# itxtx/normalizing-flows-study

Measured on AMD Instinct MI355X. Metric: log_prob samples/sec/GPU + test-NLL match; RealNVP d=2 and MAF d=63, higher is better.
Workload: dtype fp32

## Files before the change

### include/nfx.h

```cpp
#ifndef NFX_H
#define NFX_H

#include <stddef.h>
#include <stdint.h>

#ifdef __cplusplus
extern "C" {
#endif

#define NFX_ABI_VERSION 3

#define NFX_OK 0
#define NFX_EINVAL (-1)
#define NFX_EUNSUPPORTED (-2)
#define NFX_ELAUNCH (-3)

#define NFX_FORWARD 1
#define NFX_INVERSE (-1)

#define NFX_MAF_INVERSE 0
#define NFX_IAF_FORWARD 1
#define NFX_MAF_FORWARD 2
#define NFX_IAF_INVERSE 3

typedef struct NfxMlpRaw {
    const float* w[4];
    const float* b[4];
    const float* mask[4];
    const float* bn_w[3];
    const float* bn_b[3];
    const float* bn_rm[3];
    const float* bn_rv[3];
    float bn_eps;
    int n_layers;
} NfxMlpRaw;

int nfx_abi_version(void);
const char* nfx_last_error(void);
const char* nfx_last_kernel(void);
int nfx_debug_fill_lds(uint32_t bits, void* stream);

size_t nfx_affine_packed_floats(int d, int H);
int nfx_affine_pack(const NfxMlpRaw* s_net, const NfxMlpRaw* b_net, const float* mask, int d,
                    int H, float* packed, void* stream);
int nfx_affine_coupling(const float* packed, const float* in, float* out, float* log_det,
                        int64_t B, int d, int H, int direction, int accumulate, void* stream);
int nfx_affine_coupling_logprob(const float* packed, const float* in, float* out, float* log_det,
                                float* logp, double* sums, void* workspace, int64_t B, int d,
                                int H, int accumulate, void* stream);
#define NFX_AFFINE_AUTO 0
#define NFX_AFFINE_STREAMING 1
#define NFX_AFFINE_SMALL 2
int nfx_affine_kernel_policy(int policy);

int nfx_affine_chain_supported(int64_t B, int d, int H);
int nfx_affine_chain(const float* const* packs, int n_layers, const float* in, float* out,
                     float* log_det, int64_t B, int d, int H, int direction, int accumulate,
                     void* stream);
int nfx_affine_chain_logprob(const float* const* packs, int n_layers, const float* in, float* out,
                             float* log_det, float* logp, double* sums, void* workspace, int64_t B,
                             int d, int H, int accumulate, void* stream);
int nfx_affine_chain_sample(const float* const* packs, int n_layers, uint64_t seed, uint64_t* rng_state,
                            float* z, float* x, float* log_det, int64_t B, int d, int H, void* stream);

size_t nfx_spline_packed_floats(int d, int H, int K);
int nfx_spline_pack(const NfxMlpRaw* param_net, const float* mask, int d, int H, int K,
                    float* packed, void* stream);
int nfx_spline_coupling(const float* packed, const float* in, float* out, float* log_det,
                        int64_t B, int d, int H, int K, float bound, float min_bin_width,
                        float min_bin_height, float min_derivative, int rescale,
                        float data_min, float data_max, int direction, int accumulate,
                        void* stream);
int nfx_spline_coupling_logprob(const float* packed, const float* in, float* out, float* log_det,
                                float* logp, double* sums, void* workspace, int64_t B, int d,
                                int H, int K, float bound, float min_bin_width,
                                float min_bin_height, float min_derivative, int rescale,
                                float data_min, float data_max, int accumulate, void* stream);

int nfx_spline_chain_supported(int64_t B, int d, int H, int K);
int nfx_spline_chain(const float* const* packs, int n_layers, const float* in, float* out, float* log_det,
                     int64_t B, int d, int H, int K, float bound, float min_bin_width, float min_bin_height,
                     float min_derivative, int direction, int accumulate, void* stream);
int nfx_spline_chain_logprob(const float* const* packs, int n_layers, const float* in, float* out,
                             float* log_det, float* logp, double* sums, void* workspace, int64_t B, int d,
                             int H, int K, float bound, float min_bin_width, float min_bin_height,
                             float min_derivative, int accumulate, void* stream);
int nfx_spline_chain_sample(const float* const* packs, int n_layers, uint64_t seed, uint64_t* rng_state,
                            float* z, float* x, float* log_det, int64_t B, int d, int H, int K, float bound,
                            float min_bin_width, float min_bin_height, float min_derivative, void* stream);

int nfx_rqs_unit(const float* in, const float* widths, const float* heights,
                 const float* derivatives, float* out, float* log_det, int64_t N, int K,
                 float min_bin_width, float min_bin_height, float min_derivative, int inverse,
                 void* stream);
int nfx_rqs_unit_backward(const float* in, const float* widths, const float* heights,
                          const float* derivatives, const float* grad_out, const float* grad_log_det,
                          float* grad_in, float* grad_widths, float* grad_heights, float* grad_derivatives,
                          int64_t N, int K, float min_bin_width, float min_bin_height, float min_derivative,
                          int inverse, void* stream);

size_t nfx_arqs_packed_floats(int d, int H, int K);
int nfx_arqs_pack(const NfxMlpRaw* made, int d, int H, int K, float* packed, void* stream);
int nfx_arqs(const float* packed, const float* in, float* out, float* log_det, int64_t B, int d,
             int H, int K, float min_bin_width, float min_bin_height, float min_derivative,
             int rescale, double data_min, double data_max, int direction, int accumulate,
             void* stream);

int nfx_base_normal(uint64_t seed, uint64_t* rng_state, float* z, int64_t B, int d, void* stream);

size_t nfx_made_packed_floats(int d, int H);
int nfx_made_pack(const NfxMlpRaw* net, int d, int H, float* packed, void* stream);
int nfx_made_pack_parallel(const NfxMlpRaw* net, int d, int H, float* packed, void* stream);
int nfx_made_pack_sequential(int d, int H, float* packed, void* stream);
int nfx_made_affine(const float* packed, const float* in, float* out, float* log_det,
                    int64_t B, int d, int H, int variant, int accumulate, void* stream);
#define NFX_MADE_SEQ_AUTO 0
#define NFX_MADE_SEQ_SEGMENT 1
#define NFX_MADE_SEQ_WAVE 2
#define NFX_MADE_SEQ_PUSH 3
int nfx_made_seq_policy(int policy);
int nfx_made_affine_logprob(const float* packed, const float* in, float* out, float* log_det,
                            float* logp, double* sums, void* workspace, int64_t B, int d, int H,
                            int variant, int accumulate, void* stream);
int nfx_made_sample_supported(int d, int H, int variant);
int nfx_made_affine_sample(const float* packed, uint64_t seed, uint64_t* rng_state, float* z, float* x,
                           float* log_det, int64_t B, int d, int H, void* stream);

int nfx_made_pack_backward(const NfxMlpRaw* net, int d, int H, float* packed, void* stream);
size_t nfx_made_backward_factor_floats(int64_t B, int d, int H);
int64_t nfx_made_backward_max_batch(int d, int H);
int nfx_made_affine_backward(const float* packed, const float* in, const float* grad_out,
                             const float* grad_log_det, float* grad_in, float* factors, int64_t B,
                             int d, int H, int variant, void* stream);

int nfx_made_seq_backward(const float* packed, const float* in, const float* grad_out,
                          const float* grad_log_det, float* grad_in, float* factors, int64_t B,
                          int d, int H, int variant, void* stream);
int64_t nfx_made_factor_pitch(int64_t B);
size_t nfx_made_param_floats(int d, int H);
size_t nfx_made_wgrad_workspace_bytes(int64_t B, int d, int H);
int nfx_made_backward_weights(const float* factors, int64_t B, int d, int H,
                              const float* const* masks, float* grads, void* workspace,
                              void* stream);

size_t nfx_spline_backward_packed_floats(int d, int H, int K);
size_t nfx_spline_backward_param_floats(int d, int H, int K);
size_t nfx_spline_backward_workspace_bytes(int64_t B, int d, int H, int K);
int nfx_spline_pack_backward(const NfxMlpRaw* net, const float* mask, int d, int H, int K,
                             float* packed, void* stream);
int nfx_spline_coupling_backward(const float* packed, const float* mask, const float* in,
                                 const float* grad_out, const float* grad_log_det, float* grad_in,
                                 float* grads, void* workspace, int64_t B, int d, int H, int K,
                                 int n_transformed, float bound, float min_bin_width,
                                 float min_bin_height, float min_derivative, int direction,
                                 void* stream);

size_t nfx_affine_train_pack_floats(int d, int H);
size_t nfx_affine_train_stats_doubles(int H);
size_t nfx_affine_train_grad_doubles(int d, int H);
size_t nfx_affine_train_param_floats(int d, int H);
size_t nfx_affine_train_workspace_bytes(int64_t B, int d, int H);
int nfx_affine_train_pack(const NfxMlpRaw* s_net, const NfxMlpRaw* b_net, const float* mask,
                          const double* stats1, const double* stats2, int d, int H, float* tpack,
                          float* epack, void* stream);
int nfx_affine_train_stats(const float* tpack, const float* in, int64_t B, int d, int H, int layer,
                           double* stats, void* workspace, void* stream);
int nfx_affine_train_update_running(const double* stats1, const double* stats2,
                                    float* const* running_mean, float* const* running_var, int H,
                                    double momentum, void* stream);
int nfx_affine_train_update_running_counted(const double* stats1, const double* stats2,
                                            float* const* running_mean, float* const* running_var,
                                            int64_t* const* num_batches_tracked, int H,
                                            double momentum, void* stream);
int nfx_affine_train_backward(const float* tpack, const float* in, const float* grad_out,
                              const float* grad_log_det, float* grad_in, int64_t B, int d, int H,
                              int direction, int stage, const double* stats2, double* G,
                              void* workspace, void* stream);
int nfx_affine_train_assemble(const double* G, const double* stats1, const double* stats2, int d,
                              int H, float eps, float* grads, void* stream);
size_t nfx_affine_train_keep_floats(int64_t B, int d, int H);
int nfx_affine_train_stats_keep(const float* tpack, const float* in, int64_t B, int d, int H,
                                int layer, double* stats, void* workspace, float* keep,
                                void* stream);
int nfx_affine_train_backward_keep(const float* tpack, const float* in, const float* grad_out,
                                   const float* grad_log_det, float* grad_in, int64_t B, int d,
                                   int H, int direction, int stage, const double* stats2,
                                   double* G, void* workspace, const float* keep, void* stream);
int nfx_affine_train_output(const float* tpack, const float* in, const float* keep, float* out,
                            float* log_det, int64_t B, int d, int H, int direction, void* stream);
int nfx_affine_eval_stats(float* const* running_mean, float* const* running_var, int H,
                          double* stats1, double* stats2, void* stream);

size_t nfx_gauss_workspace_bytes(int64_t B);
int nfx_gauss_workspace_init(void* workspace, void* stream);
int nfx_gauss_logprob(const float* z, const float* log_det, float* logp, double* sums,
                      void* workspace, int64_t B, int d, void* stream);
int nfx_gauss_logprob_backward(const float* z, const float* grad_logp, float* grad_z, float* grad_log_det,
                               int64_t B, int d, void* stream);

size_t nfx_flowbn_workspace_bytes(int64_t B, int d);
int nfx_flowbn_apply(const float* in, float* out, float* log_det, const float* gamma, const float* beta,
                     const float* running_mean, const float* running_var, float eps, int64_t B, int d,
                     int direction, void* stream);
int nfx_flowbn_moments(const float* x, int64_t B, int d, double* stats, void* workspace, void* stream);
int nfx_flowbn_update_running(const double* stats, float* running_mean, float* running_var,
                              double momentum, int d, void* stream);
int nfx_flowbn_backward(const float* in, const float* grad_out, const float* grad_log_det, float* grad_in,
                        const float* gamma, const float* beta, const float* running_mean,
                        const float* running_var, float eps, float* grad_gamma, float* grad_beta,
                        int64_t B, int d, int direction, void* workspace, void* stream);


int nfx_linear_forward(const float* x, const float* w, const float* wmask, const float* b, const float* in_scale,
                       const float* post_scale, const float* post_shift, float* y, int64_t M, int K, int N,
                       int relu, void* stream);
int nfx_linear_backward_data(const float* gy, const float* w, const float* wmask, const float* act,
                             const float* out_scale, float* gx, int64_t M, int N, int K, int accumulate, void* stream);
size_t nfx_linear_workspace_bytes(int64_t M, int N, int K);
int nfx_linear_backward_weight(const float* gy, const float* x, const float* in_scale, const float* wmask, float* gw,
                               float* gb, int64_t M, int N, int K, void* workspace, void* stream);
int nfx_made_elem_forward(const float* x, const float* params, float* y, float* log_det, int64_t B, int d,
                          int variant, int accumulate, void* stream);
int nfx_made_elem_step(const float* x, const float* params, float* work, float* work_ld, int64_t B, int d, int i,
                       int variant, void* stream);
int nfx_made_elem_finish(const float* x, const float* work, const float* work_ld, float* y, float* log_det,
                         int64_t B, int d, int variant, int accumulate, void* stream);
int nfx_made_elem_backward(const float* x, const float* params, const float* gy, const float* gld, float* gparams,
                           float* gx, int64_t B, int d, int variant, void* stream);
int nfx_made_elem_seq_backward(const float* x, const float* params, const float* work, const float* lam,
                               const float* gy, const float* gld, float* out, int64_t B, int d, int variant, int mode,
                               void* stream);
int nfx_made_elem_seq_step_backward(const float* x, const float* params, const float* work, const float* work_ld,
                                    const float* lam, const float* grad_out, const float* grad_log_det,
                                    float* grad_params, float* grad_in, int64_t B, int d, int i, int variant,
                                    void* stream);
int nfx_made_elem_prefix(const float* work, float* out, int64_t B, int d, int i, void* stream);
int nfx_affine_elem_forward(const float* x, const float* s_raw, const float* b_raw, const float* mask, float* y,
                            float* log_det, int64_t B, int d, int direction, int accumulate, void* stream);
int nfx_affine_elem_backward(const float* x, const float* s_raw, const float* b_raw, const float* mask,
                             const float* gy, const float* gld, float* gs, float* gb, float* gx, int64_t B, int d,
                             int direction, void* stream);
int nfx_bn_prepare(const double* stats, const float* gamma, const float* beta, float* running_mean,
                   float* running_var, double eps, double momentum, int update_running, int N, float* mean,
                   float* invstd, float* scale, float* shift, void* stream);
int nfx_bn_apply_relu(const float* z, const float* scale, const float* shift, float* h, int64_t M, int N,
                      void* stream);
size_t nfx_bn_workspace_bytes(int64_t M, int N);
int nfx_bn_backward_sums(const float* g, const float* z, const float* mean, const float* invstd, double* sums,
                         int64_t M, int N, void* workspace, void* stream);
int nfx_bn_backward_apply(const float* g, const float* z, const float* mean, const float* invstd,
                          const float* gamma, const double* sums, const double* count, int train, float* gz,
                          int64_t M, int N, void* stream);
int nfx_arqs_step(const float* xr, const float* params, float* state, float* log_det, const float* gld, float* lam,
                  float* gparams, float* gx, int64_t B, int d, int K, int i, int direction, int mode,
                  float min_bin_width, float min_bin_height, float min_derivative, void* stream);
int nfx_arqs_bounds(const float* in, const float* bounds, float* out, int64_t B, int d, int mode, void* stream);
int nfx_spline_elem_forward(const float* x, const float* params, const float* mask, float* y, float* log_det,
                            int64_t B, int d, int K, float bound, float min_bin_width, float min_bin_height,
                            float min_derivative, int direction, int accumulate, void* stream);
int nfx_spline_elem_backward(const float* x, const float* params, const float* mask, const float* gy,
                             const float* gld, float* gparams, float* gx, int64_t B, int d, int K, float bound,
                             float min_bin_width, float min_bin_height, float min_derivative, int direction,
                             void* stream);
int nfx_spline_elem_forward_bounded(const float* x, const float* params, const float* mask, const float* bounds,
                                    float* y, float* log_det, int64_t B, int d, int K, float bound,
                                    float min_bin_width, float min_bin_height, float min_derivative, int direction,
                                    int accumulate, void* stream);
int nfx_spline_elem_backward_bounded(const float* x, const float* params, const float* mask, const float* bounds,
                                     const float* gy, const float* gld, float* gparams, float* gx, int64_t B, int d,
                                     int K, float bound, float min_bin_width, float min_bin_height,
                                     float min_derivative, int direction, void* stream);
int nfx_spline_rescale(const float* x, const float* bounds, float* xr, int64_t B, int d, float bound, void* stream);

size_t nfx_cnf_packed_floats(int d, int H);
int nfx_cnf_pack(const float* w1, const float* b1, const float* w2, const float* b2, const float* w3,
                 const float* b3, int d, int H, float* packed, void* stream);
int nfx_cnf_supported(int64_t B, int d, int H);
int nfx_cnf_integrate(const float* packed, const float* in, float* out, float* log_det, int64_t B, int d,
                      int H, float t_begin, float t_end, float step_size, int accumulate, void* stream);

int nfx_cnf_backward_supported(int64_t B, int d, int H);
size_t nfx_cnf_backward_packed_floats(int d, int H);
size_t nfx_cnf_trajectory_floats(int64_t B, int d, float t_begin, float t_end, float step_size);
size_t nfx_cnf_backward_workspace_floats(int64_t B, int d, int H);
size_t nfx_cnf_backward_slots(int64_t B, int d, int H);
size_t nfx_cnf_backward_block_threads(int64_t B, int d, int H);
int nfx_cnf_pack_backward(const float* w1, const float* b1, const float* w2, const float* b2, const float* w3,
                          const float* b3, int d, int H, float* packed, void* stream);
int nfx_cnf_integrate_save(const float* packed, const float* in, float* out, float* log_det, float* traj,
                           int64_t B, int d, int H, float t_begin, float t_end, float step_size, int accumulate,
                           void* stream);
int nfx_cnf_backward(const float* packed, const float* w1, const float* w2, const float* w3, const float* in,
                     const float* traj, const float* gy, const float* gld, float* gx, float* gw1, float* gb1,
                     float* gw2, float* gb2, float* gw3, float* gb3, float* workspace, int64_t B, int d, int H,
                     float t_begin, float t_end, float step_size, void* stream);

#define NFX_RESIDUAL_RELU 0
#define NFX_RESIDUAL_ELU 1
#define NFX_RESIDUAL_LEAKY_RELU 2
#define NFX_RESIDUAL_TANH 3
size_t nfx_residual_packed_floats(int d, int H);
int nfx_residual_supported(int64_t B, int d, int H, int activation);
int nfx_residual_pack(const float* w1, const float* b1, const float* u1, const float* v1, float c1, const float* w2,
                      const float* b2, const float* u2, const float* v2, float c2, const float* w3, const float* b3,
                      const float* u3, const float* v3, float c3, int d, int H, float* packed, void* stream);
int nfx_residual_flow(const float* packed, const float* in, float* out, float* log_det, int64_t B, int d, int H,
                      int activation, int direction, int neumann_terms, int max_iter, float tol, int accumulate,
                      void* stream);

int nfx_residual_backward_supported(int64_t B, int d, int H, int activation);
size_t nfx_residual_backward_packed_floats(int d, int H);
size_t nfx_residual_backward_workspace_floats(int64_t B, int d, int H);
size_t nfx_residual_backward_slots(int64_t B, int d, int H);
size_t nfx_residual_backward_block_threads(int64_t B, int d, int H);
int nfx_residual_pack_backward(const float* w1, const float* b1, const float* u1, const float* v1, float c1,
                               const float* w2, const float* b2, const float* u2, const float* v2, float c2,
                               const float* w3, const float* b3, const float* u3, const float* v3, float c3, int d,
                               int H, float* packed, void* stream);
int nfx_residual_backward(const float* packed, const float* z, const float* gy, const float* gld, float* gx,
                          float* gw1, float* gb1, float* gw2, float* gb2, float* gw3, float* gb3, float* workspace,
                          int64_t B, int d, int H, int activation, int direction, int neumann_terms, void* stream);

#define NFX_NAF_RELU 0
#define NFX_NAF_ELU 1
#define NFX_NAF_LEAKY_RELU 2
#define NFX_NAF_GELU 3
#define NFX_NAF_LAYER_NORM 1
#define NFX_NAF_RESIDUAL(l) (2 << (l))
typedef struct NfxNafLayer {
    const float* weight;
    const float* bias;
    const float* mask;
    const float* ln_weight;
    const float* ln_bias;
    float ln_eps;
    int residual;
} NfxNafLayer;
size_t nfx_naf_packed_floats(int d, int n_hidden, const int* widths);
int nfx_naf_supported(int64_t B, int d, int n_hidden, const int* widths, int activation, int flags);
int nfx_naf_pack(const NfxNafLayer* layers, int d, int n_hidden, const int* widths, float* packed, void* stream);
int nfx_naf_flow(const float* packed, const float* in, float* out, float* log_det, int64_t B, int d, int n_hidden,
                 const int* widths, int activation, int flags, float clamp_alpha, float clamp_log_scale,
                 int direction, int accumulate, void* stream);

typedef struct NfxNafLayerGrad {
    float* weight;
    float* bias;
    float* ln_weight;
    float* ln_bias;
} NfxNafLayerGrad;
int nfx_naf_backward_supported(int64_t B, int d, int n_hidden, const int* widths, int activation, int flags);
size_t nfx_naf_backward_packed_floats(int d, int n_hidden, const int* widths);
int nfx_naf_pack_backward(const NfxNafLayer* layers, int d, int n_hidden, const int* widths, float* packed,
                          void* stream);
size_t nfx_naf_backward_slots(int64_t B, int d, int n_hidden, const int* widths);
size_t nfx_naf_backward_block_threads(int64_t B, int d, int n_hidden, const int* widths);
size_t nfx_naf_backward_workspace_floats(int64_t B, int d, int n_hidden, const int* widths);
int nfx_naf_backward(const float* packed, const NfxNafLayer* layers, const float* x, const float* gz,
                     const float* gld, float* gx, const NfxNafLayerGrad* grads, float* workspace, int64_t B, int d,
                     int n_hidden, const int* widths, int activation, int flags, float clamp_alpha,
                     float clamp_log_scale, void* stream);

int nfx_lowrank_supported(int64_t B, int dim, int n_layers);
size_t nfx_lowrank_record_floats(int dim);
int nfx_lowrank_pack_planar(const float* w, const float* u_hat, const float* b, int dim, int max_iter, float tol,
                            float* record, void* stream);
int nfx_lowrank_pack_radial(const float* z0, const float* alpha_hat, const float* beta_hat, int dim, int max_iter,
                            float tol, float* record, void* stream);
int nfx_lowrank_pack_sylvester(const float* v, const float* R, const float* b, int dim, int num_householder,
                               int num_transforms, int max_iter, float tol, float* record, void* stream);
int nfx_lowrank_stack(const float* image, int n_layers, const float* x, float* out, float* log_det, int64_t B,
                      int dim, int direction, int accumulate, void* stream);

int nfx_lrbwd_supported(int64_t B, int dim, int n_layers, int direction);
size_t nfx_lrbwd_max_layers(int dim);
size_t nfx_lrbwd_chunk_rows(int dim);
size_t nfx_lrbwd_slots(int64_t B, int dim, int n_layers);
size_t nfx_lrbwd_workspace_floats(int64_t B, int dim, int n_layers);
int nfx_lrbwd_stack(const float* image, int n_layers, const float* point, const float* gv, const float* gld, float* gx,
                    float* workspace, int64_t B, int dim, int direction, void* stream);
int nfx_lrbwd_param_grads(const float* workspace, int64_t B, int dim, int n_layers, int layer, int kind,
                          const float* p0, const float* p1, const float* p2, float* g0, float* g1, float* g2,
                          int num_householder, int num_transforms, void* stream);

#ifdef __cplusplus
}
#endif

#endif
```

### normalizing-flows-study_amd/csrc/nfx_affine_kernel.h

```cpp
#pragma once
#include <type_traits>
#include <utility>

#include "nfx_common.h"

namespace nfx {

__host__ __device__ constexpr int up4(int v) { return (v + 3) & ~3; }

struct AffineLayout {
    int d, HT, KS1;
    int w1, b1, w2, b2, w3, b3, net, mask, total;
    int s;
};

constexpr uint32_t kAffineLiveElide = 0x100u;
struct AffineSplit {
    int w1, b1, b2, w3, b3, w2s, net, mask, ok, total;
};

__host__ __device__ constexpr AffineSplit affine_split(int d, int HT) {
    AffineSplit S{};
    int o = 0;
    S.w1 = o; o += HT * ((d + 1) / 2) * 64;
    S.b1 = o; o += HT * 32;
    S.b2 = o; o += HT * 32;
    S.w3 = o; o += d * HT * 32;
    S.b3 = o; o += up4(d);
    S.w2s = o; o += HT * 2 * HT * 768;
    S.net = o;
    S.mask = 2 * o;
    S.ok = S.mask + up4(d);
    S.total = S.ok + 4;
    return S;
}

__host__ __device__ constexpr bool affine_has_split(int d, int HT) { return d <= 8 && HT <= 2; }

__host__ __device__ constexpr AffineLayout affine_layout(int d, int HT) {
    AffineLayout L{};
    L.d = d;
    L.HT = HT;
    L.KS1 = (d + 1) / 2;
    int o = 0;
    L.w1 = o; o += HT * L.KS1 * 64;
    L.b1 = o; o += HT * 32;
    L.w2 = o; o += HT * HT * 16 * 64;
    L.b2 = o; o += HT * 32;
    if (d <= 8) {
        L.w3 = o; o += d * HT * 32;
        L.b3 = o; o += up4(d);
    } else {
        const int NJ = (d + 31) / 32;
        L.w3 = o; o += NJ * HT * 1024;
        L.b3 = o; o += NJ * 32;
    }
    L.net = o;
    L.mask = 2 * o;
    L.total = 2 * o + up4(d);
    L.s = L.total;
    if (affine_has_split(d, HT)) L.total += affine_split(d, HT).total;
    return L;
}

template <int D>
__device__ __forceinline__ void load_row(const float* __restrict__ p, float (&v)[D]) {
    if constexpr (D == 2) {
        float2 t = *reinterpret_cast<const float2*>(p);
        v[0] = t.x; v[1] = t.y;
    } else if constexpr (D == 4) {
        float4 t = *reinterpret_cast<const float4*>(p);
        v[0] = t.x; v[1] = t.y; v[2] = t.z; v[3] = t.w;
    } else {
#pragma unroll
        for (int j = 0; j < D; ++j) v[j] = p[j];
    }
}

template <int D>
__device__ __forceinline__ void store_row(float* __restrict__ p, const float (&v)[D]) {
    if constexpr (D == 2) {
        *reinterpret_cast<float2*>(p) = make_float2(v[0], v[1]);
    } else if constexpr (D == 4) {
        *reinterpret_cast<float4*>(p) = make_float4(v[0], v[1], v[2], v[3]);
    } else {
#pragma unroll
        for (int j = 0; j < D; ++j) p[j] = v[j];
    }
}

template <int HT, int D, int TILES = 2>
__device__ __forceinline__ void affine_net(const float* __restrict__ P, const AffineLayout& L,
                                           const float (&xb)[2][(D + 1) / 2], float (&res)[D]) {
    constexpr int KS1 = (D + 1) / 2;
    const int lane = lane_id(), h = lane >> 5;

    f32x16 h1[HT][2];
#pragma unroll
    for (int ht = 0; ht < HT; ++ht) {
        f32x16 a0, a1;
        load_bias16_x2(P + L.b1 + ht * 32, h, a0, a1);
#pragma unroll
        for (int ks = 0; ks < KS1; ++ks) {
            const float w = P[L.w1 + (ht * KS1 + ks) * 64 + lane];
            a0 = mfma32(w, xb[0][ks], a0);
            if constexpr (TILES == 2) a1 = mfma32(w, xb[1][ks], a1);
        }
#pragma unroll
        for (int r = 0; r < 16; ++r) {
            a0[r] = trelu(a0[r]);
            if constexpr (TILES == 2) a1[r] = trelu(a1[r]);
        }
        h1[ht][0] = a0;
        h1[ht][1] = a1;
    }

    float part[D][2];
#pragma unroll
    for (int j = 0; j < D; ++j) part[j][0] = part[j][1] = 0.f;
    const f32x4* wg = reinterpret_cast<const f32x4*>(P + L.w2) + lane;
#pragma unroll
    for (int hto = 0; hto < HT; ++hto) {
        f32x16 a0, a1;
        load_bias16_x2(P + L.b2 + hto * 32, h, a0, a1);
#pragma unroll
        for (int kt = 0; kt < HT; ++kt) {
#pragma unroll
            for (int rq = 0; rq < 4; ++rq) {
                const f32x4 w = wg[a_quad(a_tile(hto, kt, HT), rq) * 64];
#pragma unroll
                for (int rr = 0; rr < 4; ++rr) {
                    a0 = mfma32(w[rr], h1[kt][0][4 * rq + rr], a0);
                    if constexpr (TILES == 2) a1 = mfma32(w[rr], h1[kt][1][4 * rq + rr], a1);
                }
            }
        }
#pragma unroll
        for (int j = 0; j < D; ++j) {
            const f32x16 w3 = load_bias16(P + L.w3 + (j * HT + hto) * 32, h);
#pragma unroll
            for (int r = 0; r < 16; ++r) {
                part[j][0] = fmaf(w3[r], trelu(a0[r]), part[j][0]);
                if constexpr (TILES == 2) part[j][1] = fmaf(w3[r], trelu(a1[r]), part[j][1]);
            }
        }
    }
#pragma unroll
    for (int j = 0; j < D; ++j)
        res[j] = tclamp(halves_sum(part[j][0], part[j][1]) + P[L.b3 + j], -10.f, 10.f);
}

#ifndef NFX_SPLIT_TERMS
#define NFX_SPLIT_TERMS 6
#endif
typedef __bf16 bf16x8 __attribute__((ext_vector_type(8)));
typedef uint32_t u32x4 __attribute__((ext_vector_type(4)));

__device__ __forceinline__ f32x16 mfma_bf16(u32x4 a, u32x4 b, f32x16 c) {
    return __builtin_amdgcn_mfma_f32_32x32x16_bf16(__builtin_bit_cast(bf16x8, a), __builtin_bit_cast(bf16x8, b), c,
                                                    0, 0, 0);
}

__device__ __forceinline__ void split3(float x, uint32_t& u0, uint32_t& u1, uint32_t& u2) {
    u0 = __float_as_uint(x) & 0xffff0000u;
    const float r1 = x - __uint_as_float(u0);
    u1 = __float_as_uint(r1) & 0xffff0000u;
    u2 = __float_as_uint(r1 - __uint_as_float(u1));
}

__device__ __forceinline__ uint32_t pack_bf16(uint32_t lo, uint32_t hi) {
    return __builtin_amdgcn_perm(hi, lo, 0x07060302u);
}

__device__ __forceinline__ void split_block(const f32x16& a, int half, u32x4 (&xp)[3]) {
#pragma unroll
    for (int q = 0; q < 4; ++q) {
        uint32_t l0, l1, l2, h0, h1, h2;
        split3(a[8 * half + 2 * q], l0, l1, l2);
        split3(a[8 * half + 2 * q + 1], h0, h1, h2);
        xp[0][q] = pack_bf16(l0, h0);
        xp[1][q] = pack_bf16(l1, h1);
        xp[2][q] = pack_bf16(l2, h2);
    }
}

template <class F, int... I>
__device__ __forceinline__ void static_for_seq(F&& f, std::integer_sequence<int, I...>) {
    (f(std::integral_constant<int, I>{}), ...);
}
template <int N, class F>
__device__ __forceinline__ void static_for(F&& f) {
    static_for_seq(f, std::make_integer_sequence<int, N>{});
}

#if NFX_SPLIT_TERMS == 8
constexpr int kSplitTermW[8] = {2, 1, 2, 1, 0, 1, 0, 0}, kSplitTermX[8] = {1, 2, 0, 1, 2, 0, 1, 0};
#else
constexpr int kSplitTermW[6] = {2, 1, 0, 1, 0, 0}, kSplitTermX[6] = {0, 1, 2, 0, 1, 0};
#endif

template <int HT, int D, int TILES, bool LIVE>
__device__ __forceinline__ void affine_nets_split_pipe(const float* __restrict__ S, const AffineSplit& SL,
                                                       const float (&xb)[2][(D + 1) / 2], float (&sv)[D],
                                                       float (&bv)[D], uint32_t live_idx) {
    constexpr int KS1 = (D + 1) / 2;
    constexpr int NJ = LIVE ? (D + 1) / 2 : D;
    constexpr int NS = 2 * TILES;
    constexpr int KB = 2 * HT;
    constexpr int NT = NFX_SPLIT_TERMS;
    constexpr int NM = NT * HT;
    constexpr int NG = KB * NM;
    constexpr int NFI = 16 * HT;
    constexpr int NQ = 3 * HT;
    constexpr int WG0 = (NM - NQ) / 2;
    constexpr int L1G = (KB - 2) * NM;
    constexpr int L1P = L1G >= 2 ? L1G - 2 : 0;
    constexpr int HB0 = NM / 2;
    const int lane = lane_id(), h = lane >> 5;

    const float* Sn[NS];
    const u32x4* w2n[NS];
    f32x16 h1[NS][HT];
    uint32_t u[NS * KB][3][8];
    u32x4 xp[NS * KB][3];
    u32x4 w[NS * KB][HT][3];
    f32x16 hi[NS][HT], lo[NS][HT];
    f32x4 w3q[NS][HT][NJ][4];
    float r1[NS * KB][8], tf[NS][NFI];
    float part[2][NJ][2];
    int w3row[NJ];
#pragma unroll
    for (int j = 0; j < NJ; ++j) w3row[j] = (LIVE ? (int)((live_idx >> (4 * j)) & 7u) : j) * HT * 32;
#pragma unroll
    for (int n = 0; n < 2; ++n)
#pragma unroll
        for (int j = 0; j < NJ; ++j) part[n][j][0] = part[n][j][1] = 0.f;

    auto base = [&](int s) __attribute__((always_inline)) {
        Sn[s] = S + (s / TILES) * SL.net + opaque_zero();
        w2n[s] = reinterpret_cast<const u32x4*>(Sn[s] + SL.w2s) + lane;
    };
    auto l1_bias = [&](int s) __attribute__((always_inline)) {
#pragma unroll
        for (int ht = 0; ht < HT; ++ht) h1[s][ht] = load_bias16(Sn[s] + SL.b1 + ht * 32, h);
    };
    auto l1_mfma = [&](int s) __attribute__((always_inline)) {
#pragma unroll
        for (int ht = 0; ht < HT; ++ht)
#pragma unroll
            for (int ks = 0; ks < KS1; ++ks)
                h1[s][ht] = mfma32(Sn[s][SL.w1 + (ht * KS1 + ks) * 64 + lane], xb[s % TILES][ks], h1[s][ht]);
    };
    auto split_slot = [&](int b, int i) __attribute__((always_inline)) {
        const int s = b / KB, kb = b % KB, q = i / 3;
#pragma unroll
        for (int e = 2 * q; e < 2 * q + 2; ++e) {
            if (i % 3 == 0) {
                const float x = trelu(h1[s][kb >> 1][8 * (kb & 1) + e]);
                u[b][0][e] = __float_as_uint(x) & 0xffff0000u;
                r1[b][e] = x - __uint_as_float(u[b][0][e]);
            } else if (i % 3 == 1) {
                u[b][1][e] = __float_as_uint(r1[b][e]) & 0xffff0000u;
                u[b][2][e] = __float_as_uint(r1[b][e] - __uint_as_float(u[b][1][e]));
            }
        }
        if (i % 3 == 2) {
#pragma unroll
            for (int p = 0; p < 3; ++p) xp[b][p][q] = pack_bf16(u[b][p][2 * q], u[b][p][2 * q + 1]);
        }
    };
    auto w2_quad = [&](int b, int i) __attribute__((always_inline)) {
        const int s = b / KB, kb = b % KB, p = 2 - i / HT, hto = i % HT;
        w[b][hto][p] = w2n[s][((hto * KB + kb) * 3 + p) * 64];
    };
    auto w3_quads = [&](int s, int hto, int rq) __attribute__((always_inline)) {
#pragma unroll
        for (int j = 0; j < NJ; ++j)
            w3q[s][hto][j][rq] = *reinterpret_cast<const f32x4*>(Sn[s] + SL.w3 + w3row[j] + hto * 32 + 16 * h + 4 * rq);
    };
    auto fold_relu = [&](int s, int f) __attribute__((always_inline)) {
        tf[s][f] = trelu(hi[s][f / 16][f % 16] + lo[s][f / 16][f % 16]);
    };
    auto fold_fma = [&](int s, int f) __attribute__((always_inline)) {
        const int hto = f / 16, r = f % 16;
#pragma unroll
        for (int j = 0; j < NJ; ++j)
            part[s / TILES][j][s % TILES] = fmaf(w3q[s][hto][j][r / 4][r % 4], tf[s][f], part[s / TILES][j][s % TILES]);
    };
    constexpr auto fold_gap = [](int f) { return (((f | 1) + 1) * NG + NFI - 1) / NFI - 1; };
    constexpr auto w3_gap = [](int f) {
        const int g = (((f | 1) + 1) * NG + NFI - 1) / NFI - 1;
        return g >= 2 ? g - 2 : 0;
    };
    static_assert(fold_gap(NFI - 1) < NG && fold_gap(0) >= 1 && w3_gap(0) < fold_gap(0), "fold schedule");
    static_assert(WG0 >= 0 && WG0 + NQ <= NM && HB0 + HT <= NM - HT, "read schedule");
    static_assert(KB < 2 || L1G <= (KB - 1) * NM - 1, "layer 1 of the next stage precedes its first split");

    base(0);
    l1_bias(0);
#pragma unroll
    for (int i = 0; i < NQ; ++i) w2_quad(0, i);
    l1_mfma(0);
#pragma unroll
    for (int i = 0; i < 12; ++i) split_slot(0, i);

    static_for<NS>([&](auto sc) __attribute__((always_inline)) {
        constexpr int s = decltype(sc)::value;
        static_for<NG>([&](auto gc) __attribute__((always_inline)) {
            constexpr int g = decltype(gc)::value;
            constexpr int kb = g / NM, m = g % NM, b = s * KB + kb;
            constexpr int t = m / HT, hto = m % HT;
            __builtin_amdgcn_sched_barrier(0);
            if (t == NT - 1) {
                hi[s][hto] = mfma_bf16(w[b][hto][kSplitTermW[t]], xp[b][kSplitTermX[t]], hi[s][hto]);
            } else {
                lo[s][hto] = mfma_bf16(w[b][hto][kSplitTermW[t]], xp[b][kSplitTermX[t]],
                                       kb == 0 && t == 0 ? f32x16{} : lo[s][hto]);
            }
            __builtin_amdgcn_sched_barrier(0);
            if (g == 0 && s + 1 < NS) base(s + 1);
            if (b + 1 < NS * KB && m >= WG0 && m < WG0 + NQ) w2_quad(b + 1, m - WG0);
            if (kb == 0 && m >= HB0 && m < HB0 + HT)
                hi[s][m - HB0] = load_bias16(Sn[s] + SL.b2 + (m - HB0) * 32, h);
            if (s > 0) {
#pragma unroll
                for (int fq = 0; fq < NFI; fq += 4)
                    if (w3_gap(fq) == g) w3_quads(s - 1, fq / 16, (fq % 16) / 4);
            }
            if (s + 1 < NS && g == L1P) l1_bias(s + 1);
            if (s + 1 < NS && g == L1G) l1_mfma(s + 1);
            if (b + 1 < NS * KB) {
#pragma unroll
                for (int i = m * 12 / NM; i < (m + 1) * 12 / NM; ++i) split_slot(b + 1, i);
            }
            if (s > 0) {
#pragma unroll
                for (int f = 0; f < NFI; ++f)
                    if ((fold_gap(f) >= 1 ? fold_gap(f) - 1 : 0) == g) fold_relu(s - 1, f);
#pragma unroll
                for (int f = 0; f < NFI; ++f)
                    if (fold_gap(f) == g) fold_fma(s - 1, f);
            }
        });
    });
    __builtin_amdgcn_sched_barrier(0);
#pragma unroll
    for (int fq = 0; fq < NFI; fq += 4) w3_quads(NS - 1, fq / 16, (fq % 16) / 4);
#pragma unroll
    for (int f = 0; f < NFI; ++f) {
        fold_relu(NS - 1, f);
        fold_fma(NS - 1, f);
    }
    if constexpr (LIVE) {
#pragma unroll
        for (int j = 0; j < D; ++j) sv[j] = bv[j] = 0.f;
#pragma unroll
        for (int jj = 0; jj < NJ; ++jj) {
            const int o = (int)((live_idx >> (4 * jj)) & 15u);
            const float s = tclamp(halves_sum(part[0][jj][0], part[0][jj][1]) + Sn[0][SL.b3 + (o & 7)], -10.f, 10.f);
            const float b = tclamp(halves_sum(part[1][jj][0], part[1][jj][1]) + Sn[NS - 1][SL.b3 + (o & 7)], -10.f, 10.f);
#pragma unroll
            for (int j = 0; j < D; ++j) {
                sv[j] = o == j ? s : sv[j];
                bv[j] = o == j ? b : bv[j];
            }
        }
    } else {
#pragma unroll
        for (int j = 0; j < D; ++j) {
            sv[j] = tclamp(halves_sum(part[0][j][0], part[0][j][1]) + Sn[0][SL.b3 + j], -10.f, 10.f);
            bv[j] = tclamp(halves_sum(part[1][j][0], part[1][j][1]) + Sn[NS - 1][SL.b3 + j], -10.f, 10.f);
        }
    }
}

template <int KS1>
__device__ __forceinline__ bool affine_live_unit(const float (&xb)[2][KS1], const float (&mkb)[KS1]) {
    bool bad = false;
#pragma unroll
    for (int st = 0; st < 2; ++st)
#pragma unroll
        for (int ks = 0; ks < KS1; ++ks)
            bad = bad || (mkb[ks] == 1.f && (!(fabsf(xb[st][ks]) <= 1e33f) || __float_as_uint(xb[st][ks]) == 0x80000000u));
    return __builtin_amdgcn_ballot_w64(bad) == 0;
}

template <int HT, int D, int TILES = 2>
__device__ __forceinline__ void affine_net_split(const float* __restrict__ S, const AffineSplit& SL,
                                                 const float (&xb)[2][(D + 1) / 2], float (&res)[D]) {
    constexpr int KS1 = (D + 1) / 2;
    const int lane = lane_id(), h = lane >> 5;

    f32x16 h1[HT][2];
#pragma unroll
    for (int ht = 0; ht < HT; ++ht) {
        f32x16 a0, a1;
        load_bias16_x2(S + SL.b1 + ht * 32, h, a0, a1);
#pragma unroll
        for (int ks = 0; ks < KS1; ++ks) {
            const float w = S[SL.w1 + (ht * KS1 + ks) * 64 + lane];
            a0 = mfma32(w, xb[0][ks], a0);
            if constexpr (TILES == 2) a1 = mfma32(w, xb[1][ks], a1);
        }
#pragma unroll
        for (int r = 0; r < 16; ++r) {
            a0[r] = trelu(a0[r]);
            if constexpr (TILES == 2) a1[r] = trelu(a1[r]);
        }
        h1[ht][0] = a0;
        h1[ht][1] = a1;
    }

    float part[D][2];
#pragma unroll
    for (int j = 0; j < D; ++j) part[j][0] = part[j][1] = 0.f;
    auto fold = [&](int hto, const f32x16& a, int st) {
#pragma unroll
        for (int j = 0; j < D; ++j) {
            const f32x16 w3 = load_bias16(S + SL.w3 + (j * HT + hto) * 32, h);
#pragma unroll
            for (int r = 0; r < 16; ++r) part[j][st] = fmaf(w3[r], trelu(a[r]), part[j][st]);
        }
    };
    const u32x4* w2s = reinterpret_cast<const u32x4*>(S + SL.w2s) + lane;
#pragma unroll
    for (int st = 0; st < TILES; ++st) {
        u32x4 xp[2 * HT][3];
#pragma unroll
        for (int kb = 0; kb < 2 * HT; ++kb) split_block(h1[kb >> 1][st], kb & 1, xp[kb]);
        const u32x4* w2 = w2s + opaque_zero();
#pragma unroll
        for (int hto = 0; hto < HT; ++hto) {
            f32x16 hi = load_bias16(S + SL.b2 + hto * 32 + opaque_zero(), h), lo = {};
#pragma unroll
            for (int kb = 0; kb < 2 * HT; ++kb) {
                const int g = (hto * 2 * HT + kb) * 3;
                const u32x4 w[3] = {w2[g * 64], w2[(g + 1) * 64], w2[(g + 2) * 64]};
#if NFX_SPLIT_TERMS == 8
                lo = mfma_bf16(w[2], xp[kb][1], lo);
                lo = mfma_bf16(w[1], xp[kb][2], lo);
#endif
                lo = mfma_bf16(w[2], xp[kb][0], lo);
                lo = mfma_bf16(w[1], xp[kb][1], lo);
                lo = mfma_bf16(w[0], xp[kb][2], lo);
                lo = mfma_bf16(w[1], xp[kb][0], lo);
                lo = mfma_bf16(w[0], xp[kb][1], lo);
                hi = mfma_bf16(w[0], xp[kb][0], hi);
            }
            fold(hto, hi + lo, st);
        }
    }
#pragma unroll
    for (int j = 0; j < D; ++j)
        res[j] = tclamp(halves_sum(part[j][0], part[j][1]) + S[SL.b3 + j], -10.f, 10.f);
}

__host__ __device__ constexpr bool affine_split_piped(int HT, int D) { return HT == 2 && D <= 4; }

template <int HT, int D, int TILES, bool PIPE>
__device__ __forceinline__ void affine_nets_split(const float* __restrict__ S, const AffineSplit& SL,
                                                  const float* __restrict__ Pg, const AffineLayout& L,
                                                  const float (&xb)[2][(D + 1) / 2], float (&sv)[D], float (&bv)[D],
                                                  bool live = false, uint32_t live_idx = 0) {
    constexpr int KS1 = (D + 1) / 2;
    const bool wok = S[SL.ok] != 0.f;
    const float xs = S[SL.ok + 1];
    bool fast[2];
#pragma unroll
    for (int st = 0; st < 2; ++st) {
        bool bad = false;
#pragma unroll
        for (int ks = 0; ks < KS1; ++ks) bad = bad || !(fabsf(xb[st][ks]) <= xs);
        fast[st] = wok && __builtin_amdgcn_ballot_w64(bad) == 0;
    }
    if constexpr (PIPE) {
        bool full = !live;
        if (live) {
            affine_nets_split_pipe<HT, D, TILES, true>(S, SL, xb, sv, bv, live_idx);
            bool zero = true;
#pragma unroll
            for (int j = 0; j < D; ++j) zero = zero && fabsf(sv[j]) < 1e-30f;
            full = __builtin_amdgcn_ballot_w64(zero) != 0;
        }
        if (full) affine_nets_split_pipe<HT, D, TILES, false>(S, SL, xb, sv, bv, 0u);
    } else {
        affine_net_split<HT, D, TILES>(S, SL, xb, sv);
        __builtin_amdgcn_sched_barrier(0);
        affine_net_split<HT, D, TILES>(S + SL.net, SL, xb, bv);
    }
    if (!(fast[0] && (TILES == 1 || fast[1]))) {
        __builtin_amdgcn_sched_barrier(0);
        const float* P = Pg + opaque_zero();
        float s2[D], b2[D];
        affine_net<HT, D, TILES>(P, L, xb, s2);
        __builtin_amdgcn_sched_barrier(0);
        affine_net<HT, D, TILES>(P + L.net, L, xb, b2);
        if (!fast[lane_id() >> 5]) {
#pragma unroll
            for (int j = 0; j < D; ++j) {
                sv[j] = s2[j];
                bv[j] = b2[j];
            }
        }
    }
}

template <int HT, int D, int DIR, bool LOGP>
__global__ __launch_bounds__(256) void affine_coupling_kernel(
    const float* __restrict__ packed, const float* __restrict__ in, float* __restrict__ out,
    float* __restrict__ logdet, int64_t B, int accumulate, int64_t nchunks,
    float* __restrict__ logp, double* __restrict__ partials, double* __restrict__ sums, float cgauss) {
    constexpr AffineLayout L = affine_layout(D, HT);
    constexpr int KS1 = L.KS1;
    constexpr bool SPLIT = affine_has_split(D, HT);
    constexpr AffineSplit SL = affine_split(D, HT);
    constexpr int MASK = SPLIT ? SL.mask : L.mask;
    extern __shared__ f32x4 lds4[];
    {
        const f32x4* src = reinterpret_cast<const f32x4*>(packed + (SPLIT ? L.s : 0));
        for (int i = threadIdx.x; i < (SPLIT ? SL.total : L.total) / 4; i += 256) lds4[i] = src[i];
    }
    __syncthreads();
    const float* sm = reinterpret_cast<const float*>(lds4);

    const int lane = lane_id(), h = lane >> 5, col = lane & 31;
    const int64_t nwaves = (int64_t)gridDim.x * 4;
    float mk[D], mkb[KS1];
#pragma unroll
    for (int j = 0; j < D; ++j) mk[j] = sm[MASK + j];
#pragma unroll
    for (int ks = 0; ks < KS1; ++ks) mkb[ks] = (2 * ks + h < D) ? sm[MASK + 2 * ks + h] : 0.f;
    const int64_t wv = (int64_t)blockIdx.x * 4 + (threadIdx.x >> 6);
    const int64_t F = nchunks / nwaves, R = nchunks - F * nwaves;
    const bool split = 2 * R <= nwaves;
    const int64_t nfull = split ? F : F + (wv < R ? 1 : 0);
    const bool half = split && wv < 2 * R;
    const int64_t half_base = F * nwaves * 64 + wv * 32;

    struct Fetch {
        float xb[2][KS1];
        float xr[D];
        float ldin;
    };
    auto fetch = [&](int64_t u, Fetch& f) {
        const int64_t base = u < nfull ? (wv + u * nwaves) * 64 : half_base;
        const int nsamp = u < nfull ? 64 : (u == nfull && half ? 32 : 0);
#pragma unroll
        for (int st = 0; st < 2; ++st) {
            const int64_t s = base + 32 * st + col;
#pragma unroll
            for (int ks = 0; ks < KS1; ++ks) {
                const int k = 2 * ks + h;
                f.xb[st][ks] = (32 * st + col < nsamp && k < D && s < B) ? in[s * D + k] : 0.f;
            }
        }
        const int64_t so = base + lane;
        if (lane < nsamp && so < B) {
            load_row<D>(in + so * D, f.xr);
            f.ldin = accumulate ? logdet[so] : 0.f;
        } else {
#pragma unroll
            for (int j = 0; j < D; ++j) f.xr[j] = 0.f;
            f.ldin = 0.f;
        }
    };

    double lpacc = 0.0;
    auto unit = [&](auto tiles_c, int64_t base, const Fetch& cur) {
        constexpr int TILES = decltype(tiles_c)::value;
        const float* smi = sm + opaque_zero();
        float xb[2][KS1];
#pragma unroll
        for (int st = 0; st < 2; ++st) {
#pragma unroll
            for (int ks = 0; ks < KS1; ++ks) xb[st][ks] = cur.xb[st][ks] * mkb[ks];
        }

        float sv[D], bv[D];
        if constexpr (SPLIT) {
            affine_nets_split<HT, D, TILES, false>(smi, SL, packed, L, xb, sv, bv);
        } else {
            affine_net<HT, D, TILES>(smi, L, xb, sv);
            affine_net<HT, D, TILES>(smi + L.net, L, xb, bv);
        }

        const int64_t so = base + lane;
        if (lane < 32 * TILES && so < B) {
#pragma clang fp contract(off)
            float y[D];
            float ld = 0.f;
#pragma unroll
            for (int j = 0; j < D; ++j) {
                const float m = mk[j], om = 1.f - m;
                const float xa = cur.xr[j] * m;
                float t;
                if constexpr (DIR < 0) {
                    t = (cur.xr[j] - bv[j]) * exp_fast(-sv[j]);
                    ld = ld + om * (-sv[j]);
                } else {
                    t = cur.xr[j] * exp_fast(sv[j]) + bv[j];
                    ld = ld + om * sv[j];
                }
                const float v = xa + om * t;
                y[j] = nonfinite(v) ? 0.f : v;
            }
            if (nonfinite(ld)) ld = 0.f;
            store_row<D>(out + so * D, y);
            const float ldt = accumulate ? cur.ldin + ld : ld;
            logdet[so] = ldt;
            if constexpr (LOGP) {
                float m = gauss_sq0(y[0]);
#pragma unroll
                for (int j = 1; j < D; ++j) m = gauss_sq(m, y[j]);
                const float lp = gauss_lp(m, cgauss, ldt);
                logp[so] = lp;
                lpacc += (double)lp;
            }
        }
    };

    Fetch cur;
    fetch(0, cur);
    for (int64_t u = 0; u < nfull; ++u) {
        Fetch nxt;
        fetch(u + 1, nxt);
        unit(std::integral_constant<int, 2>{}, (wv + u * nwaves) * 64, cur);
        cur = nxt;
    }
    if (half) unit(std::integral_constant<int, 1>{}, half_base, cur);
    if constexpr (LOGP) {
        logp_commit<256>(lpacc, partials, sums, B);
    }
}


constexpr int kWideWaves = 4;

template <int HT>
__device__ __forceinline__ void wide_net(const float* __restrict__ P, const AffineLayout& L, const float* xt, int S,
                                         const float* __restrict__ mask, int d, f32x16 (&res)[2]) {
    const int lane = lane_id(), h = lane >> 5, col = lane & 31;
    f32x16 h1[HT];
#pragma unroll
    for (int ht = 0; ht < HT; ++ht) h1[ht] = load_bias16(P + L.b1 + ht * 32, h);
    for (int ks = 0; ks < L.KS1; ++ks) {
        const int k = 2 * ks + h;
        const float xb = k < d ? xt[col * S + k] * mask[k] : 0.f;
#pragma unroll
        for (int ht = 0; ht < HT; ++ht) h1[ht] = mfma32(P[L.w1 + (ht * L.KS1 + ks) * 64 + lane], xb, h1[ht]);
    }
#pragma unroll
    for (int ht = 0; ht < HT; ++ht)
#pragma unroll
        for (int r = 0; r < 16; ++r) h1[ht][r] = trelu(h1[ht][r]);
    f32x16 h2[HT];
#pragma unroll
    for (int hto = 0; hto < HT; ++hto) {
        f32x16 a = load_bias16(P + L.b2 + hto * 32, h);
#pragma unroll
        for (int kt = 0; kt < HT; ++kt)
#pragma unroll
            for (int rq = 0; rq < 4; ++rq) {
                const f32x4 w = *reinterpret_cast<const f32x4*>(P + L.w2 + (a_quad(a_tile(hto, kt, HT), rq) * 64 + lane) * 4);
#pragma unroll
                for (int rr = 0; rr < 4; ++rr) a = mfma32(w[rr], h1[kt][4 * rq + rr], a);
            }
#pragma unroll
        for (int r = 0; r < 16; ++r) a[r] = trelu(a[r]);
        h2[hto] = a;
    }
    const int NJ = (d + 31) / 32;
#pragma unroll
    for (int j = 0; j < 2; ++j) {
        if (j < NJ) {
            f32x16 a = load_bias16(P + L.b3 + j * 32, h);
#pragma unroll
            for (int kt = 0; kt < HT; ++kt)
#pragma unroll
                for (int rq = 0; rq < 4; ++rq) {
                    const f32x4 w = *reinterpret_cast<const f32x4*>(P + L.w3 + (a_quad(a_tile(j, kt, HT), rq) * 64 + lane) * 4);
#pragma unroll
                    for (int rr = 0; rr < 4; ++rr) a = mfma32(w[rr], h2[kt][4 * rq + rr], a);
                }
#pragma unroll
            for (int r = 0; r < 16; ++r) a[r] = tclamp(a[r], -10.f, 10.f);
            res[j] = a;
        } else {
            res[j] = f32x16{};
        }
    }
}

template <int HT, int DIR, bool LOGP>
__global__ __launch_bounds__(64 * kWideWaves) void affine_wide_kernel(
    const float* __restrict__ packed, const float* __restrict__ in, float* __restrict__ out,
    float* __restrict__ logdet, int64_t B, int d, int accumulate, int64_t ntiles,
    float* __restrict__ logp, double* __restrict__ partials, double* __restrict__ sums, float cgauss) {
    const AffineLayout L = affine_layout(d, HT);
    const int S = d | 1;
    extern __shared__ f32x4 lds4[];
    const int wave = __builtin_amdgcn_readfirstlane(threadIdx.x >> 6);
    float* xt = reinterpret_cast<float*>(lds4) + wave * 32 * S;
    const int lane = lane_id(), h = lane >> 5, col = lane & 31;
    const float* mask = packed + L.mask;
    double lpacc = 0.0;
    for (int64_t t = (int64_t)blockIdx.x * kWideWaves + wave; t < ntiles; t += (int64_t)gridDim.x * kWideWaves) {
        const int64_t base = t * 32;
        const int rows = (int)(B - base < 32 ? B - base : 32);
        const float* src = in + base * d;
        for (int i = lane; i < 32 * d; i += 64) {
            const int r = i / d, c = i - r * d;
            xt[r * S + c] = r < rows ? src[i] : 0.f;
        }
        const float ldin = (accumulate && lane < rows) ? logdet[base + lane] : 0.f;
        wave_lds_sync();
        const float* Pw = packed + opaque_zero();
        f32x16 sv[2], bv[2];
        wide_net<HT>(Pw, L, xt, S, mask, d, sv);
        wide_net<HT>(Pw + L.net, L, xt, S, mask, d, bv);
        float ldp = 0.f;
        {
#pragma clang fp contract(off)
#pragma unroll
            for (int j = 0; j < 2; ++j)
#pragma unroll
                for (int r = 0; r < 16; ++r) {
                    const int dim = 32 * j + crow(r, h);
                    if (dim < d) {
                        float* px = xt + col * S + dim;
                        const float xv = *px, m = mask[dim], om = 1.f - m;
                        float tv;
                        if constexpr (DIR < 0) {
                            tv = (xv - bv[j][r]) * exp_fast(-sv[j][r]);
                            ldp = ldp + om * (-sv[j][r]);
                        } else {
                            tv = xv * exp_fast(sv[j][r]) + bv[j][r];
                            ldp = ldp + om * sv[j][r];
                        }
                        const float v = xv * m + om * tv;
                        *px = nonfinite(v) ? 0.f : v;
                    }
                }
        }
        float ld = halves_sum(ldp, ldp);
        if (nonfinite(ld)) ld = 0.f;
        wave_lds_sync();
        float* dst = out + base * d;
        for (int i = lane; i < rows * d; i += 64) {
            const int r = i / d, c = i - r * d;
            dst[i] = xt[r * S + c];
        }
        if (lane < rows) {
            const float ldt = accumulate ? ldin + ld : ld;
            logdet[base + lane] = ldt;
            if constexpr (LOGP) {
                float m = gauss_sq0(xt[lane * S]);
                for (int c = 1; c < d; ++c) m = gauss_sq(m, xt[lane * S + c]);
                const float lp = gauss_lp(m, cgauss, ldt);
                logp[base + lane] = lp;
                lpacc += (double)lp;
            }
        }
        wave_lds_sync();
    }
    if constexpr (LOGP) {
        logp_commit<64 * kWideWaves>(lpacc, partials, sums, B);
    }
}

typedef void (*affine_kernel_t)(const float*, const float*, float*, float*, int64_t, int, int64_t,
                                float*, double*, double*, float);

template <int HT>
affine_kernel_t affine_pick_ht(int d, int dir, bool logp);

template <int HT>
affine_kernel_t affine_pick(int d, int dir, bool logp) {
    return pick_range<1, 8>(d, [=](auto D) -> affine_kernel_t {
        if (dir > 0) return affine_coupling_kernel<HT, D(), 1, false>;
        return logp ? affine_coupling_kernel<HT, D(), -1, true> : affine_coupling_kernel<HT, D(), -1, false>;
    });
}

int affine_split_pack(float* packed, int d, int H, hipStream_t s);

}
```

### normalizing-flows-study_amd/csrc/nfx_made.hip

```cpp
#include "nfx_made_kernel.h"
#include "nfx_made_wide_kernel.h"
#include <atomic>
#include <cstdlib>

#include "nfx_made_seqs_kernel.h"
#include "nfx_pack.h"

namespace nfx {

__global__ void made_pack_kernel(NfxMlpRaw net, int d, int H, float* packed) {
    const int HT = (H + 31) / 32;
    const MadeLayout L = made_layout(d, HT);
    const int Hp = L.Hp, G1 = 4 * L.NKC;
    for (int i = blockIdx.x * blockDim.x + threadIdx.x; i < L.total; i += gridDim.x * blockDim.x) {
        if (i >= L.s_deg) continue;
        float v = 0.f;
        if (i < L.b1) {
            int t = i - L.w1, rr = t & 3, lane = (t >> 2) & 63, g = (t >> 8) % G1, ht = (t >> 8) / G1;
            int row = 32 * ht + (lane & 31), col = 2 * (4 * g + rr) + (lane >> 5);
            v = (row < H && col < d) ? mlp_weight(net, 0, d, row, col) : 0.f;
        } else if (i < L.w2) {
            int row = acc_vec_row(i - L.b1);
            v = row < H ? mlp_bias(net, 0, row) : 0.f;
        } else if (i < L.b2 || (i >= L.w3 && i < L.b3)) {
            const int layer = i < L.b2 ? 1 : 2;
            const ATileElem e = a_tile_elem(i - (layer == 1 ? L.w2 : L.w3));
            int row = 32 * (e.tile / HT) + e.row, col = 32 * (e.tile % HT) + e.k;
            v = (row < H && col < H) ? mlp_weight(net, layer, H, row, col) : 0.f;
        } else if (i < L.w3 || (i >= L.b3 && i < L.w4)) {
            const int layer = i < L.w3 ? 1 : 2;
            int row = acc_vec_row(i - (layer == 1 ? L.b2 : L.b3));
            v = row < H ? mlp_bias(net, layer, row) : 0.f;
        } else if (i < L.b4) {
            const ATileElem e = a_tile_elem(i - L.w4);
            int jw = e.tile / HT, which = jw & 1, j = jw >> 1;
            int orow = 32 * j + e.row, col = 32 * (e.tile % HT) + e.k;
            v = (orow < d && col < H) ? mlp_weight(net, 3, H, which * d + orow, col) : 0.f;
        } else if (i < L.par_total) {
            int t = i - L.b4, jw = t >> 5, which = jw & 1, j = jw >> 1;
            int orow = 32 * j + acc_vec_row(t & 31);
            v = orow < d ? mlp_bias(net, 3, which * d + orow) : 0.f;
        } else if (i < L.s_b1) {
            int t = i - L.s_w1t, ii = t / Hp, a = t % Hp;
            v = (ii < d && a < H) ? mlp_weight(net, 0, d, a, ii) : 0.f;
        } else if (i < L.s_w2) {
            int a = i - L.s_b1;
            v = a < H ? mlp_bias(net, 0, a) : 0.f;
        } else if (i < L.s_b2 || (i >= L.s_w3 && i < L.s_b3)) {
            const int layer = i < L.s_b2 ? 1 : 2;
            int t = i - (layer == 1 ? L.s_w2 : L.s_w3), a = t / Hp, b = t % Hp;
            v = (a < H && b < H) ? mlp_weight(net, layer, H, a, b) : 0.f;
        } else if (i < L.s_w3 || (i >= L.s_b3 && i < L.s_w4)) {
            const int layer = i < L.s_w3 ? 1 : 2;
            int a = i - (layer == 1 ? L.s_b2 : L.s_b3);
            v = a < H ? mlp_bias(net, layer, a) : 0.f;
        } else if (i < L.s_b4) {
            int t = i - L.s_w4, row = t / Hp, a = t % Hp;
            v = (row < 2 * d && a < H) ? mlp_weight(net, 3, H, row, a) : 0.f;
        } else if (i < L.s_deg) {
            int row = i - L.s_b4;
            v = row < 2 * d ? mlp_bias(net, 3, row) : 0.f;
        }
        packed[i] = v;
    }
}

constexpr int kLiveThreads = 1024;

__global__ __launch_bounds__(kLiveThreads) void made_live_kernel(NfxMlpRaw net, int d, int H, float* packed) {
    const int HT = (H + 31) / 32;
    const MadeLayout L = made_layout(d, HT);
    {
        __shared__ int deg[256];
        const int Hp = L.Hp;
        for (int a0 = 0; a0 < Hp; a0 += kLiveThreads / 16) {
            const int a = a0 + (threadIdx.x >> 4), q = threadIdx.x & 15;
            int n = 0;
            if (a < H && net.mask[0]) {
                const float* row = net.mask[0] + (size_t)a * d;
#pragma unroll 4
                for (int j = q; j < d; j += 16) n += row[j] != 0.f ? 1 : 0;
            }
            n += __shfl_xor(n, 1);
            n += __shfl_xor(n, 2);
            n += __shfl_xor(n, 4);
            n += __shfl_xor(n, 8);
            if (q == 0 && a < Hp) deg[a] = a < H ? (net.mask[0] ? n - 1 : 0) : 1000000000;
        }
        __syncthreads();
        for (int a = threadIdx.x; a < Hp; a += kLiveThreads) {
            const int da = deg[a];
            int rank = 0;
            for (int b = 0; b < Hp; ++b) rank += (deg[b] < da || (deg[b] == da && b < a)) ? 1 : 0;
            packed[L.s_deg + a] = (float)da;
            packed[L.s_deg + Hp + rank] = (float)da;
            packed[L.s_deg + 2 * Hp + rank] = (float)a;
        }
    }
    int* nk = reinterpret_cast<int*>(packed);
    for (int i = threadIdx.x; i < 3 * HT + L.NJ; i += kLiveThreads) nk[L.nk1 + i] = 0;
    __shared__ double red[256];
    const int rows[4] = {H, H, H, 2 * d}, cols[4] = {d, H, H, H};
    const double tsafe = block_mlp_tsafe(net, 4, rows, cols, 1.0e37, red);
    if (threadIdx.x == 0) packed[L.tsafe] = (float)fmin(tsafe, 3.0e38);
}

__global__ __launch_bounds__(256) void made_extent_kernel(int d, int H, float* packed) {
    const int HT = (H + 31) / 32;
    const MadeLayout L = made_layout(d, HT);
    int* nk = reinterpret_cast<int*>(packed);
    const int n1 = HT * 4 * L.NKC, n23 = HT * HT * 4, n4 = L.NJ * 2 * HT * 4;
    const int lane = lane_id();
    for (int gi = blockIdx.x * 4 + (threadIdx.x >> 6); gi < n1 + 2 * n23 + n4; gi += gridDim.x * 4) {
        int off, word, ext;
        if (gi < n1) {
            const int ht = gi / (4 * L.NKC), g = gi % (4 * L.NKC);
            off = L.w1 + gi * 256;
            word = L.nk1 + ht;
            ext = g / 4 + 1;
        } else if (gi < n1 + 2 * n23) {
            const int t = (gi - n1) % n23, layer = (gi - n1) / n23;
            off = (layer == 0 ? L.w2 : L.w3) + t * 256;
            word = (layer == 0 ? L.nk2 : L.nk3) + t / (HT * 4);
            ext = (t % (HT * 4)) / 4 + 1;
        } else {
            const int t = gi - n1 - 2 * n23;
            off = L.w4 + t * 256;
            word = L.nk4 + t / (2 * HT * 4);
            ext = (t % (HT * 4)) / 4 + 1;
        }
        const f32x4 v = *reinterpret_cast<const f32x4*>(packed + off + 4 * lane);
        const bool nzl = v[0] != 0.f || v[1] != 0.f || v[2] != 0.f || v[3] != 0.f;
        if (__ballot(nzl) != 0 && lane == 0) atomicMax(&nk[word], ext);
    }
}

template <int HT>
made_seqs_kernel_t made_seqs_pick_ht(int variant, bool logp) {
    if (variant == NFX_MAF_FORWARD) return made_seqs_kernel<HT, NFX_MAF_FORWARD, false>;
    return logp ? made_seqs_kernel<HT, NFX_IAF_INVERSE, true> : made_seqs_kernel<HT, NFX_IAF_INVERSE, false>;
}
template made_seqs_kernel_t made_seqs_pick_ht<1>(int, bool);
template made_seqs_kernel_t made_seqs_pick_ht<2>(int, bool);

template <int HT, int VAR>
static made_seq_kernel_t seq_var() {
    return made_seq_kernel<HT, VAR>;
}

template <int HT>
made_seq_kernel_t made_seq_pick_ht(int variant) {
    return variant == NFX_MAF_FORWARD ? seq_var<HT, NFX_MAF_FORWARD>() : seq_var<HT, NFX_IAF_INVERSE>();
}
template made_seq_kernel_t made_seq_pick_ht<1>(int);
template made_seq_kernel_t made_seq_pick_ht<2>(int);
template made_seq_kernel_t made_seq_pick_ht<3>(int);
template made_seq_kernel_t made_seq_pick_ht<4>(int);

static made_par_kernel_t pick_par(int HT, bool wlds, int variant) {
    return pick_range<1, 4>(HT, [=](auto HT_) { return made_pick_ht<HT_()>(wlds, variant); });
}

static made_par_kernel_t pick_tile(int HT, bool wlds, int variant, bool logp) {
    return pick_range<1, 4>(HT, [=](auto HT_) { return made_tile_pick_ht<HT_()>(wlds, variant, logp); });
}

static made_seq_kernel_t pick_seq(int HT, int variant) {
    return pick_range<1, 4>(HT, [=](auto HT_) { return made_seq_pick_ht<HT_()>(variant); });
}

int made_big_launch(const float* packed, const float* in, float* out, float* log_det, int64_t B, int d, int H,
                    int variant, int accumulate, hipStream_t s);

constexpr size_t kLdsBytes = 160 * 1024;
constexpr int kTileMaxD = 64;

}

using namespace nfx;

extern "C" size_t nfx_made_packed_floats(int d, int H) {
    if (d <= 0 || H <= 0) return 0;
    return (size_t)made_layout(d, (H + 31) / 32).total;
}

namespace nfx {
int made_pack_seqp(int d, int H, float* packed, hipStream_t s);
static int made_pack_seq(int d, int H, float* packed, hipStream_t s) {
    const int HT = (H + 31) / 32;
    if (HT > 2) return NFX_OK;
    if (HT == 1) made_seqs_image_kernel<1><<<64, 256, 0, s>>>(packed, d, H);
    else made_seqs_image_kernel<2><<<64, 256, 0, s>>>(packed, d, H);
    int rc = check_launch("made_seqs_image_kernel");
    if (rc) return rc;
    if (HT == 1) made_seqs_chunk_kernel<1><<<1, 64, 0, s>>>(packed, d, H);
    else made_seqs_chunk_kernel<2><<<1, 64, 0, s>>>(packed, d, H);
    rc = check_launch("made_seqs_chunk_kernel");
    if (rc) return rc;
    return made_pack_seqp(d, H, packed, s);
}
}

extern "C" int nfx_made_pack_parallel(const NfxMlpRaw* net, int d, int H, float* packed, void* stream) {
    if (!net || !packed) return set_error(NFX_EINVAL, "made_pack: null pointer");
    if (d <= 0 || d > 4096 || H <= 0 || H > 256)
        return set_error(NFX_EUNSUPPORTED, "made_pack: d=%d H=%d outside d<=4096, H<=256", d, H);
    if (net->n_layers != 4) return set_error(NFX_EINVAL, "made_pack: MADE has 4 masked layers (got %d)", net->n_layers);
    for (int l = 0; l < 4; ++l)
        if (!net->w[l]) return set_error(NFX_EINVAL, "made_pack: layer %d weight is null", l);
    const int total = (int)nfx_made_packed_floats(d, H);
    int blocks = (total + 255) / 256;
    if (blocks > 2048) blocks = 2048;
    made_pack_kernel<<<blocks, 256, 0, (hipStream_t)stream>>>(*net, d, H, packed);
    int rc = check_launch("made_pack_kernel");
    if (rc) return rc;
    made_live_kernel<<<1, kLiveThreads, 0, (hipStream_t)stream>>>(*net, d, H, packed);
    rc = check_launch("made_live_kernel");
    if (rc) return rc;
    {
        const int HT = (H + 31) / 32;
        const MadeLayout L = made_layout(d, HT);
        const int groups = HT * 4 * L.NKC + 2 * HT * HT * 4 + L.NJ * 2 * HT * 4;
        made_extent_kernel<<<(groups + 3) / 4, 256, 0, (hipStream_t)stream>>>(d, H, packed);
    }
    return check_launch("made_extent_kernel");
}

extern "C" int nfx_made_pack_sequential(int d, int H, float* packed, void* stream) {
    if (!packed) return set_error(NFX_EINVAL, "made_pack_sequential: null pointer");
    if (d <= 0 || d > 4096 || H <= 0 || H > 256)
        return set_error(NFX_EUNSUPPORTED, "made_pack_sequential: d=%d H=%d outside d<=4096, H<=256", d, H);
    return made_pack_seq(d, H, packed, (hipStream_t)stream);
}

extern "C" int nfx_made_pack(const NfxMlpRaw* net, int d, int H, float* packed, void* stream) {
    const int rc = nfx_made_pack_parallel(net, d, H, packed, stream);
    if (rc) return rc;
    return made_pack_seq(d, H, packed, (hipStream_t)stream);
}

namespace nfx {
int made_seqw_launch(const float* packed, const float* in, float* out, float* log_det, int64_t B, int d, int H,
                     int variant, int accumulate, float* logp, double* partials, double* sums, bool fused,
                     int* grid_out, hipStream_t s);
int made_seqp_launch(const float* packed, const float* in, float* out, float* log_det, int64_t B, int d, int H,
                     int variant, int accumulate, float* logp, double* partials, double* sums, bool fused,
                     hipStream_t s);
}

static std::atomic<int>& made_seq_policy() {
    static std::atomic<int> v{[] {
        const char* e = getenv("NFX_MADE_SEQ_POLICY");
        return e ? atoi(e) : NFX_MADE_SEQ_AUTO;
    }()};
    return v;
}

namespace nfx {
int made_seq_policy_get() { return made_seq_policy().load(std::memory_order_relaxed); }
}

static bool tile_path(int d, int HT, int variant) {
    return (variant == NFX_MAF_INVERSE || variant == NFX_IAF_FORWARD) && d > 0 && d <= kTileMaxD && HT >= 1 && HT <= 4;
}

struct TileConfig {
    int nw;
    bool wlds;
    size_t lds;
};
static TileConfig tile_config(const MadeLayout& L, int64_t ntiles, bool fused) {
    int nw = 8;
    if (!fused && ntiles < 4 * (int64_t)num_cus()) nw = (int)((ntiles + num_cus() - 1) / num_cus());
    const size_t wbytes = (size_t)L.par_total * sizeof(float);
    const size_t tiles = nw * 32 * (size_t)kTileStride * sizeof(float);
    const bool wlds = nw == 8 && wbytes + tiles <= kLdsBytes;
    return {nw, wlds, (wlds ? wbytes : 0) + tiles};
}

static int made_launch(const float* packed, const float* in, float* out, float* log_det, int64_t B,
                       int d, int H, int variant, int accumulate, float* logp, double* sums,
                       void* workspace, hipStream_t s) {
    const bool fused = sums != nullptr;
    if (B < 0 || d <= 0 || H <= 0) return set_error(NFX_EINVAL, "made_affine: bad shape");
    if (d > 4096 || H > 256) return set_error(NFX_EUNSUPPORTED, "made_affine: d=%d H=%d outside d<=4096, H<=256", d, H);
    if (variant < NFX_MAF_INVERSE || variant > NFX_IAF_INVERSE)
        return set_error(NFX_EINVAL, "made_affine: unknown variant %d", variant);
    const int HT = (H + 31) / 32;
    if (HT > 4) {
        if (fused) return set_error(NFX_EUNSUPPORTED, "made_affine_logprob: no fused log_prob for H=%d > 128", H);
        if (B == 0) return NFX_OK;
        if (!packed || !in || !out || !log_det) return set_error(NFX_EINVAL, "made_affine: null pointer");
        if (in == out) return set_error(NFX_EINVAL, "made_affine: in and out must not alias");
        return made_big_launch(packed, in, out, log_det, B, d, H, variant, accumulate, s);
    }
    const MadeLayout L = made_layout(d, HT);
    const bool parallel = variant == NFX_MAF_INVERSE || variant == NFX_IAF_FORWARD;
    const size_t wide_lds_bytes = (size_t)wide_lds(L, HT).total * sizeof(float);
    const bool wide = parallel && d > kTileMaxD && HT <= 2 && wide_lds_bytes <= kLdsBytes;
    const bool seqs = (variant == NFX_MAF_FORWARD || variant == NFX_IAF_INVERSE) && HT <= 2;
    if (fused && !((variant == NFX_MAF_INVERSE && (d <= kTileMaxD || wide)) || (variant == NFX_IAF_INVERSE && seqs)))
        return set_error(NFX_EUNSUPPORTED,
                         "made_affine_logprob: fused log_prob needs MAF inverse with d <= %d or H <= 64, "
                         "or IAF inverse with H <= 64", kTileMaxD);
    if (fused && B > 0 && (!logp || !workspace)) return set_error(NFX_EINVAL, "made_affine_logprob: null logp/workspace");
    if (B == 0) return fused ? gauss_finish(reinterpret_cast<double*>(workspace), 0, sums, 0, s) : NFX_OK;
    if (!packed || !in || !out || !log_det) return set_error(NFX_EINVAL, "made_affine: null pointer");
    if (in == out) return set_error(NFX_EINVAL, "made_affine: in and out must not alias");
    double* partials = reinterpret_cast<double*>(workspace);
    if (wide) {
        const int64_t nchunks = (B + 63) / 64;
        const int nw = nchunks < (int64_t)kWideWaves * num_cus() ? 4 : kWideWaves;
        const size_t lds_nw = (size_t)wide_lds(L, HT, nw).total * sizeof(float);
        made_par_kernel_t k = HT == 1 ? made_wide_pick_ht<1>(variant, fused, nw) : made_wide_pick_ht<2>(variant, fused, nw);
        int rc = prepare_lds((const void*)k, lds_nw);
        if (rc) return rc;
        int grid = resident_grid((const void*)k, 64 * nw, lds_nw, (nchunks + nw - 1) / nw);
        if (grid > kMaxPartials) grid = kMaxPartials;
        k<<<grid, 64 * nw, lds_nw, s>>>(packed, in, out, log_det, B, d, accumulate, nchunks, logp, partials,
                                        sums, gauss_const(d));
        return check_launch("made_wide_kernel");
    }
    if (tile_path(d, HT, variant)) {
        const int64_t ntiles = (B + 31) / 32;
        const TileConfig c = tile_config(L, ntiles, fused);
        made_par_kernel_t k = pick_tile(HT, c.wlds, variant, fused);
        if (!k) return set_error(NFX_EUNSUPPORTED, "made_affine: no kernel for H=%d", H);
        int rc = prepare_lds((const void*)k, c.lds);
        if (rc) return rc;
        int grid = resident_grid((const void*)k, 64 * c.nw, c.lds, (ntiles + c.nw - 1) / c.nw);
        if (grid > kMaxPartials) grid = kMaxPartials;
        k<<<grid, 64 * c.nw, c.lds, s>>>(packed, in, out, log_det, B, d, accumulate, ntiles, logp, partials, sums,
                                         gauss_const(d));
        return check_launch("made_tile_kernel");
    }
    if (variant == NFX_MAF_INVERSE || variant == NFX_IAF_FORWARD) {
        const size_t wbytes = (size_t)L.par_total * sizeof(float);
        const size_t stage8 = 8 * (size_t)kStageFloats * sizeof(float);
        const bool wlds = wbytes + stage8 <= kLdsBytes;
        made_par_kernel_t k = pick_par(HT, wlds, variant);
        if (!k) return set_error(NFX_EUNSUPPORTED, "made_affine: no kernel for H=%d", H);
        const int threads = wlds ? 512 : 256;
        const size_t lds = wlds ? wbytes + stage8 : 4 * (size_t)kStageFloats * sizeof(float);
        int rc = prepare_lds((const void*)k, lds);
        if (rc) return rc;
        const int64_t nchunks = (B + 63) / 64;
        const int nw = threads / 64;
        const int grid = resident_grid((const void*)k, threads, lds, (nchunks + nw - 1) / nw);
        k<<<grid, threads, lds, s>>>(packed, in, out, log_det, B, d, accumulate, nchunks, nullptr, nullptr, nullptr,
                                     0.f);
        return check_launch("made_parallel_kernel");
    }
    const int seq_pol = made_seq_policy().load(std::memory_order_relaxed);
    const bool push_auto = seq_pol == NFX_MADE_SEQ_AUTO && d > 32 && B <= 4096 * (int64_t)num_cus() / 256;
    if (seqs && (seq_pol == NFX_MADE_SEQ_PUSH || push_auto) && L.ps > 0)
        return made_seqp_launch(packed, in, out, log_det, B, d, H, variant, accumulate, logp, partials, sums, fused, s);
    if (seqs && (seq_pol == NFX_MADE_SEQ_PUSH || seq_pol == NFX_MADE_SEQ_WAVE || (seq_pol == NFX_MADE_SEQ_AUTO && B <= 2048 * (int64_t)num_cus() / 256))) {
        int grid = 0;
        return made_seqw_launch(packed, in, out, log_det, B, d, H, variant, accumulate, logp, partials, sums, fused,
                                &grid, s);
    }
    if (seqs) {
        made_seqs_kernel_t k = HT == 1 ? made_seqs_pick_ht<1>(variant, fused) : made_seqs_pick_ht<2>(variant, fused);
        const size_t lds = (size_t)seqs_lds(L.Hp).total * sizeof(float);
        int rc = prepare_lds((const void*)k, lds);
        if (rc) return rc;
        const int threads = kSeqsThreads;
        int grid = resident_grid((const void*)k, threads, lds, (B + 4 * kSeqsWaves - 1) / (4 * kSeqsWaves));
        if (grid > kMaxPartials) grid = kMaxPartials;
        k<<<grid, threads, lds, s>>>(packed, in, out, log_det, B, d, H, accumulate, logp, partials, sums,
                                     gauss_const(d));
        return check_launch("made_seqs_kernel");
    }
    made_seq_kernel_t k = pick_seq(HT, variant);
    if (!k) return set_error(NFX_EUNSUPPORTED, "made_affine: no sequential kernel for H=%d", H);
    const size_t lds = 2 * 64 * (size_t)(L.Hp + 4) * sizeof(float);
    int rc = prepare_lds((const void*)k, lds);
    if (rc) return rc;
    const int64_t grid = (B + 63) / 64;
    k<<<(unsigned)grid, 64, lds, s>>>(packed, in, out, log_det, B, d, H, accumulate);
    return check_launch("made_seq_kernel");
}

extern "C" int nfx_made_seq_policy(int policy) {
    if (policy < 0) return made_seq_policy().load();
    if (policy > NFX_MADE_SEQ_PUSH) return set_error(NFX_EINVAL, "made_seq_policy: unknown policy %d", policy);
    return made_seq_policy().exchange(policy);
}

extern "C" int nfx_made_affine(const float* packed, const float* in, float* out, float* log_det,
                               int64_t B, int d, int H, int variant, int accumulate, void* stream) {
    return made_launch(packed, in, out, log_det, B, d, H, variant, accumulate, nullptr, nullptr, nullptr,
                       (hipStream_t)stream);
}

extern "C" int nfx_made_affine_logprob(const float* packed, const float* in, float* out, float* log_det,
                                       float* logp, double* sums, void* workspace, int64_t B, int d,
                                       int H, int variant, int accumulate, void* stream) {
    if (!sums) return set_error(NFX_EINVAL, "made_affine_logprob: null sums");
    return made_launch(packed, in, out, log_det, B, d, H, variant, accumulate, logp, sums, workspace,
                       (hipStream_t)stream);
}

extern "C" int nfx_made_sample_supported(int d, int H, int variant) {
    return (H > 0 && tile_path(d, (H + 31) / 32, variant) && variant == NFX_IAF_FORWARD) ? 1 : 0;
}

extern "C" int nfx_made_affine_sample(const float* packed, uint64_t seed, uint64_t* rng_state, float* z, float* x,
                                      float* log_det, int64_t B, int d, int H, void* stream) {
    if (B < 0 || d <= 0 || H <= 0) return set_error(NFX_EINVAL, "made_affine_sample: bad shape");
    if (!nfx_made_sample_supported(d, H, NFX_IAF_FORWARD))
        return set_error(NFX_EUNSUPPORTED, "made_affine_sample: d=%d H=%d outside the tile kernel (d <= %d, H <= 128)",
                         d, H, kTileMaxD);
    if (B == 0) return NFX_OK;
    if (!packed || !rng_state || !z || !x || !log_det) return set_error(NFX_EINVAL, "made_affine_sample: null pointer");
    if (z == x) return set_error(NFX_EINVAL, "made_affine_sample: z and x must not alias");
    const int HT = (H + 31) / 32;
    const MadeLayout L = made_layout(d, HT);
    const int64_t ntiles = (B + 31) / 32;
    const TileConfig c = tile_config(L, ntiles, false);
    made_sample_kernel_t k =
        pick_range<1, 4>(HT, [=](auto HT_) { return made_tile_sample_pick_ht<HT_()>(c.wlds); });
    int rc = prepare_lds((const void*)k, c.lds);
    if (rc) return rc;
    int grid = resident_grid((const void*)k, 64 * c.nw, c.lds, (ntiles + c.nw - 1) / c.nw);
    if (grid > kMaxPartials) grid = kMaxPartials;
    k<<<grid, 64 * c.nw, c.lds, (hipStream_t)stream>>>(packed, nullptr, x, log_det, B, d, 0, ntiles, nullptr, nullptr,
                                                       nullptr, 0.f, MadeDraw{seed, rng_state, z});
    return check_launch("made_tile_kernel");
}
```

### normalizing-flows-study_amd/csrc/nfx_made_kernel.h

```cpp
#pragma once
#include "nfx_common.h"
#include "nfx_rng.h"

namespace nfx {

struct MadeLayout {
    int d, HT, Hp, NKC, NJ;
    int w1, b1, w2, b2, w3, b3, w4, b4;
    int par_total;
    int s_w1t, s_b1, s_w2, s_b2, s_w3, s_b3, s_w4, s_b4, s_deg;
    int nk1, nk2, nk3, nk4, tsafe;
    int t4, t3, t2, t1;
    int rimg;
    int sw1, sw4, sb4;
    int ctab;
    int ps, pw4, pw1, pb4, pw23, ptb, ptab;
    int total;
};

__host__ __device__ constexpr int made_up4(int v) { return (v + 3) & ~3; }

__host__ __device__ constexpr int seqs_w4_stride(int Hp) { return 2 * Hp + 4; }
constexpr int kSeqsPadRows = 64;
__host__ __device__ constexpr int seqs_max_chunks(int d, int Hp) { return d / 8 + 2 * Hp + 8; }
constexpr int kSeqpMaxS = 16;
__host__ __device__ constexpr int seqp_slots(int d, int HT) {
    return (HT <= 2 && d <= 64 * kSeqpMaxS) ? (d + 63) / 64 : 0;
}
__host__ __device__ constexpr int seqp_max_chunks(int d, int Hp) { return (d + 63) / 64 + 3 * Hp + 4; }

__host__ __device__ constexpr MadeLayout made_layout(int d, int HT) {
    MadeLayout L{};
    L.d = d;
    L.HT = HT;
    L.Hp = 32 * HT;
    L.NKC = (d + 31) / 32;
    L.NJ = (d + 31) / 32;
    int o = 0;
    L.w1 = o; o += HT * 4 * L.NKC * 256;
    L.b1 = o; o += HT * 32;
    L.w2 = o; o += HT * HT * 1024;
    L.b2 = o; o += HT * 32;
    L.w3 = o; o += HT * HT * 1024;
    L.b3 = o; o += HT * 32;
    L.w4 = o; o += L.NJ * 2 * HT * 1024;
    L.b4 = o; o += L.NJ * 2 * 32;
    L.par_total = o;
    L.s_w1t = o; o += made_up4(d * L.Hp);
    L.s_b1 = o; o += L.Hp;
    L.s_w2 = o; o += L.Hp * L.Hp;
    L.s_b2 = o; o += L.Hp;
    L.s_w3 = o; o += L.Hp * L.Hp;
    L.s_b3 = o; o += L.Hp;
    L.s_w4 = o; o += made_up4(2 * d * L.Hp);
    L.s_b4 = o; o += made_up4(2 * d);
    L.s_deg = o; o += 3 * L.Hp;
    L.nk1 = o; o += HT;
    L.nk2 = o; o += HT;
    L.nk3 = o; o += HT;
    L.nk4 = o; o += L.NJ;
    L.tsafe = o; o += 1;
    o = made_up4(o);
    L.t4 = o; o += HT * 2 * L.NJ * 1024;
    L.t3 = o; o += HT * HT * 1024;
    L.t2 = o; o += HT * HT * 1024;
    L.t1 = o; o += L.NKC * HT * 1024;
    L.rimg = o; o += HT <= 2 ? 2 * L.Hp * L.Hp + 5 * L.Hp : 0;
    o = made_up4(o);
    const int rows = HT <= 2 ? d + kSeqsPadRows : 0;
    L.sw1 = o; o += made_up4(rows * L.Hp);
    L.sw4 = o; o += made_up4(rows * seqs_w4_stride(L.Hp));
    L.sb4 = o; o += made_up4(2 * rows);
    L.ctab = o; o += HT <= 2 ? 8 * seqs_max_chunks(d, L.Hp) : 0;
    const int PS = seqp_slots(d, HT);
    L.ps = PS;
    L.pw4 = o; o += L.Hp * ((PS + 1) / 2) * 256;
    L.pw1 = o; o += L.Hp * ((PS + 3) / 4) * 256;
    L.pb4 = o; o += PS * 128;
    L.pw23 = o; o += PS ? 2 * L.Hp * L.Hp : 0;
    L.ptb = o; o += PS ? 4 * L.Hp : 0;
    L.ptab = o; o += PS ? 16 * seqp_max_chunks(d, L.Hp) : 0;
    L.total = o;
    return L;
}

constexpr int kStageStride = 33;
constexpr int kTileStride = 65;
constexpr int kStageFloats = 64 * kStageStride;

template <int VAR>
__device__ __forceinline__ float made_affine(float xv, float mu, float al, float& acc) {
#pragma clang fp contract(off)
    if constexpr (VAR == NFX_MAF_INVERSE) {
        const float a = tclamp(al, -3.f, 3.f);
        acc = acc + a;
        const float z = (xv - mu) * exp_fast(-a);
        return nonfinite(z) ? 0.f : z;
    } else {
        const float a = tclamp(al, -2.f, 2.f);
        const float m = tclamp(mu, -10.f, 10.f);
        acc = acc + a;
        const float y = xv * exp_fast(a) + m;
        return nonfinite(y) ? xv : y;
    }
}

__device__ __forceinline__ void stage_in(const float* __restrict__ in, int64_t base, int d, int64_t B,
                                         int dim0, float* st) {
    const int lane = lane_id();
#pragma unroll 8
    for (int i = 0; i < 32; ++i) {
        const int idx = i * 64 + lane;
        const int s = idx >> 5, dd = idx & 31;
        const int64_t row = base + s;
        const int dim = dim0 + dd;
        st[s * kStageStride + dd] = (row < B && dim < d) ? in[row * d + dim] : 0.f;
    }
}

__device__ __forceinline__ void stage_out(float* __restrict__ out, int64_t base, int d, int64_t B,
                                          int dim0, const float* st) {
    const int lane = lane_id();
#pragma unroll 8
    for (int i = 0; i < 32; ++i) {
        const int idx = i * 64 + lane;
        const int s = idx >> 5, dd = idx & 31;
        const int64_t row = base + s;
        const int dim = dim0 + dd;
        if (row < B && dim < d) out[row * d + dim] = st[s * kStageStride + dd];
    }
}


template <int HT>
__device__ __forceinline__ void made_hidden(const float* __restrict__ W, int woff, int boff,
                                            const f32x16 (&hin)[HT][2], f32x16 (&hout)[HT][2]) {
    const int lane = lane_id(), h = lane >> 5;
#pragma unroll
    for (int hto = 0; hto < HT; ++hto) {
        f32x16 a0, a1;
        load_bias16_x2(W + boff + hto * 32, h, a0, a1);
#pragma unroll
        for (int kt = 0; kt < HT; ++kt) {
#pragma unroll
            for (int rq = 0; rq < 4; ++rq) {
                const f32x4 w = *reinterpret_cast<const f32x4*>(W + woff + (a_quad(a_tile(hto, kt, HT), rq) * 64 + lane) * 4);
#pragma unroll
                for (int rr = 0; rr < 4; ++rr) {
                    a0 = mfma32(w[rr], hin[kt][0][4 * rq + rr], a0);
                    a1 = mfma32(w[rr], hin[kt][1][4 * rq + rr], a1);
                }
            }
        }
#pragma unroll
        for (int r = 0; r < 16; ++r) {
            a0[r] = trelu(a0[r]);
            a1[r] = trelu(a1[r]);
        }
        hout[hto][0] = a0;
        hout[hto][1] = a1;
    }
}

template <int HT, bool WLDS, int VAR>
__global__ __launch_bounds__(WLDS ? 512 : 256) void made_parallel_kernel(
    const float* __restrict__ packed, const float* __restrict__ in, float* __restrict__ out,
    float* __restrict__ logdet, int64_t B, int d, int accumulate, int64_t nchunks,
    float* __restrict__ , double* __restrict__ , double* __restrict__ ,
    float ) {
    constexpr int NWAVE = WLDS ? 8 : 4;
    const MadeLayout L = made_layout(d, HT);
    extern __shared__ f32x4 lds4[];
    float* lds = reinterpret_cast<float*>(lds4);
    const int wave = threadIdx.x >> 6;
    float* stg;
    if constexpr (WLDS) {
        const f32x4* src = reinterpret_cast<const f32x4*>(packed);
        for (int i = threadIdx.x; i < L.par_total / 4; i += NWAVE * 64) lds4[i] = src[i];
        stg = lds + L.par_total + wave * kStageFloats;
        __syncthreads();
    } else {
        stg = lds + wave * kStageFloats;
    }
    const int lane = lane_id(), h = lane >> 5, col = lane & 31;
    const int64_t nwaves = (int64_t)gridDim.x * NWAVE;

    for (int64_t c = (int64_t)blockIdx.x * NWAVE + wave; c < nchunks; c += nwaves) {
        const int64_t base = c * 64;
        const float* W = (WLDS ? lds : packed) + opaque_zero();

        f32x16 h1[HT][2];
#pragma unroll
        for (int ht = 0; ht < HT; ++ht) load_bias16_x2(W + L.b1 + ht * 32, h, h1[ht][0], h1[ht][1]);
        for (int kc = 0; kc < L.NKC; ++kc) {
            stage_in(in, base, d, B, 32 * kc, stg);
            wave_lds_sync();
#pragma unroll
            for (int g = 0; g < 4; ++g) {
                f32x4 w[HT];
#pragma unroll
                for (int ht = 0; ht < HT; ++ht)
                    w[ht] = *reinterpret_cast<const f32x4*>(W + L.w1 + ((ht * 4 * L.NKC + kc * 4 + g) * 64 + lane) * 4);
#pragma unroll
                for (int rr = 0; rr < 4; ++rr) {
                    const int k = 8 * g + 2 * rr + h;
                    const float b0 = stg[col * kStageStride + k];
                    const float b1 = stg[(32 + col) * kStageStride + k];
#pragma unroll
                    for (int ht = 0; ht < HT; ++ht) {
                        h1[ht][0] = mfma32(w[ht][rr], b0, h1[ht][0]);
                        h1[ht][1] = mfma32(w[ht][rr], b1, h1[ht][1]);
                    }
                }
            }
            wave_lds_sync();
        }
#pragma unroll
        for (int ht = 0; ht < HT; ++ht) {
#pragma unroll
            for (int r = 0; r < 16; ++r) {
                h1[ht][0][r] = trelu(h1[ht][0][r]);
                h1[ht][1][r] = trelu(h1[ht][1][r]);
            }
        }
        f32x16 h2[HT][2];
        made_hidden<HT>(W, L.w2, L.b2, h1, h2);
        made_hidden<HT>(W, L.w3, L.b3, h2, h1);

        float acc0 = 0.f, acc1 = 0.f;
        for (int j = 0; j < L.NJ; ++j) {
            f32x16 mu0, mu1, al0, al1;
            load_bias16_x2(W + L.b4 + (j * 2 + 0) * 32, h, mu0, mu1);
            load_bias16_x2(W + L.b4 + (j * 2 + 1) * 32, h, al0, al1);
#pragma unroll
            for (int kt = 0; kt < HT; ++kt) {
#pragma unroll
                for (int rq = 0; rq < 4; ++rq) {
                    const f32x4 wm = *reinterpret_cast<const f32x4*>(
                        W + L.w4 + (a_quad(a_tile(j * 2 + 0, kt, HT), rq) * 64 + lane) * 4);
                    const f32x4 wa = *reinterpret_cast<const f32x4*>(
                        W + L.w4 + (a_quad(a_tile(j * 2 + 1, kt, HT), rq) * 64 + lane) * 4);
#pragma unroll
                    for (int rr = 0; rr < 4; ++rr) {
                        const float b0 = h1[kt][0][4 * rq + rr], b1 = h1[kt][1][4 * rq + rr];
                        mu0 = mfma32(wm[rr], b0, mu0);
                        mu1 = mfma32(wm[rr], b1, mu1);
                        al0 = mfma32(wa[rr], b0, al0);
                        al1 = mfma32(wa[rr], b1, al1);
                    }
                }
            }
            stage_in(in, base, d, B, 32 * j, stg);
            wave_lds_sync();
#pragma unroll
            for (int r = 0; r < 16; ++r) {
                const int row = crow(r, h);
                if (32 * j + row < d) {
                    float* p0 = stg + col * kStageStride + row;
                    float* p1 = stg + (32 + col) * kStageStride + row;
                    *p0 = made_affine<VAR>(*p0, mu0[r], al0[r], acc0);
                    *p1 = made_affine<VAR>(*p1, mu1[r], al1[r], acc1);
                }
            }
            wave_lds_sync();
            stage_out(out, base, d, B, 32 * j, stg);
            wave_lds_sync();
        }
        float s = halves_sum(acc0, acc1);
        const int64_t so = base + lane;
        if (so < B) {
            float ld;
            if constexpr (VAR == NFX_MAF_INVERSE) {
                ld = -s;
                if (nonfinite(ld)) ld = 0.f;
                ld = tclamp(ld, -100.f, 100.f);
            } else {
                ld = s;
                if (nonfinite(ld)) ld = 0.f;
                ld = tclamp(ld, -50.f, 50.f);
            }
            logdet[so] = accumulate ? logdet[so] + ld : ld;
        }
    }
}


template <int HT, int VAR>
__global__ __launch_bounds__(64) void made_seq_kernel(
    const float* __restrict__ packed, const float* __restrict__ in, float* __restrict__ out,
    float* __restrict__ logdet, int64_t B, int d, int H, int accumulate) {
    constexpr int Hp = 32 * HT;
    constexpr int RS = Hp + 4;
    const MadeLayout L = made_layout(d, HT);
    extern __shared__ f32x4 lds4[];
    float* h1s = reinterpret_cast<float*>(lds4);
    float* h2s = h1s + 64 * RS;
    const int lane = threadIdx.x;
    const int64_t s = (int64_t)blockIdx.x * 64 + lane;
    const bool valid = s < B;
    const float* P = packed;

    float pre1[Hp], h3[Hp];
#pragma unroll
    for (int a = 0; a < Hp; ++a) {
        pre1[a] = P[L.s_b1 + a];
        h3[a] = 0.f;
        h1s[lane * RS + a] = 0.f;
        h2s[lane * RS + a] = 0.f;
    }
    float ld = 0.f;
    bool poison = false;
    int p = 0;
    const float* ord = P + L.s_deg;

    for (int i = 0; i < d; ++i) {
        float mu = 0.f, al = 0.f;
        const float* w_mu = P + L.s_w4 + (size_t)i * Hp;
        const float* w_al = P + L.s_w4 + (size_t)(d + i) * Hp;
#pragma unroll
        for (int a = 0; a < Hp; ++a) {
            mu = fmaf(w_mu[a], h3[a], mu);
            al = fmaf(w_al[a], h3[a], al);
        }
        mu = mu + P[L.s_b4 + i];
        al = al + P[L.s_b4 + d + i];
        if (poison) { mu = __builtin_nanf(""); al = mu; }
        const float xin = valid ? in[s * d + i] : 0.f;
        float xi;
        if constexpr (VAR == NFX_MAF_FORWARD) {
            const float a = tclamp(al, -3.f, 3.f);
            xi = xin * exp_fast(a) + mu;
            ld = ld + a;
            if (valid) out[s * d + i] = nonfinite(xi) ? 0.f : xi;
        } else {
            const float a = tclamp(al, -2.f, 2.f);
            const float m = tclamp(mu, -10.f, 10.f);
            xi = (xin - m) * exp_fast(-a);
            ld = ld - a;
            if (valid) out[s * d + i] = nonfinite(xi) ? xin : xi;
        }
        if (nonfinite(xi)) poison = true;
        const float* w1c = P + L.s_w1t + (size_t)i * Hp;
#pragma unroll
        for (int a = 0; a < Hp; ++a) pre1[a] = fmaf(w1c[a], xi, pre1[a]);
        int q = p;
        while (q < H && (int)ord[Hp + q] == i) ++q;
        if (q > p) {
            for (int k = p; k < q; ++k) {
                const int a = (int)ord[2 * Hp + k];
                float v = 0.f;
#pragma unroll
                for (int b = 0; b < Hp; ++b) v = (b == a) ? pre1[b] : v;
                h1s[lane * RS + a] = trelu(v);
            }
            for (int k = p; k < q; ++k) {
                const int a = (int)ord[2 * Hp + k];
                const float* w = P + L.s_w2 + (size_t)a * Hp;
                float v = 0.f;
#pragma unroll
                for (int b = 0; b < Hp; b += 4) {
                    const f32x4 hv = *reinterpret_cast<const f32x4*>(h1s + lane * RS + b);
                    v = fmaf(w[b], hv[0], v);
                    v = fmaf(w[b + 1], hv[1], v);
                    v = fmaf(w[b + 2], hv[2], v);
                    v = fmaf(w[b + 3], hv[3], v);
                }
                h2s[lane * RS + a] = trelu(v + P[L.s_b2 + a]);
            }
            for (int k = p; k < q; ++k) {
                const int a = (int)ord[2 * Hp + k];
                const float* w = P + L.s_w3 + (size_t)a * Hp;
                float v = 0.f;
#pragma unroll
                for (int b = 0; b < Hp; b += 4) {
                    const f32x4 hv = *reinterpret_cast<const f32x4*>(h2s + lane * RS + b);
                    v = fmaf(w[b], hv[0], v);
                    v = fmaf(w[b + 1], hv[1], v);
                    v = fmaf(w[b + 2], hv[2], v);
                    v = fmaf(w[b + 3], hv[3], v);
                }
                v = trelu(v + P[L.s_b3 + a]);
#pragma unroll
                for (int b = 0; b < Hp; ++b) h3[b] = (b == a) ? v : h3[b];
            }
            p = q;
        }
    }
    if (valid) {
        if (nonfinite(ld)) ld = 0.f;
        ld = (VAR == NFX_MAF_FORWARD) ? tclamp(ld, -100.f, 100.f) : tclamp(ld, -50.f, 50.f);
        logdet[s] = accumulate ? logdet[s] + ld : ld;
    }
}

typedef void (*made_seq_kernel_t)(const float*, const float*, float*, float*, int64_t, int, int, int);


template <int HT>
__device__ __forceinline__ void made_hidden1(const float* __restrict__ W, int woff, int boff,
                                             const f32x16 (&hin)[HT], f32x16 (&hout)[HT]) {
    const int lane = lane_id(), h = lane >> 5;
    f32x16 a[HT];
#pragma unroll
    for (int hto = 0; hto < HT; ++hto) {
        a[hto] = load_bias16(W + boff + hto * 32, h);
    }
#pragma unroll
    for (int kt = 0; kt < HT; ++kt) {
#pragma unroll
        for (int rq = 0; rq < 4; ++rq) {
            f32x4 w[HT];
#pragma unroll
            for (int hto = 0; hto < HT; ++hto)
                w[hto] = *reinterpret_cast<const f32x4*>(W + woff + (a_quad(a_tile(hto, kt, HT), rq) * 64 + lane) * 4);
#pragma unroll
            for (int rr = 0; rr < 4; ++rr) {
#pragma unroll
                for (int hto = 0; hto < HT; ++hto) a[hto] = mfma32(w[hto][rr], hin[kt][4 * rq + rr], a[hto]);
            }
        }
    }
#pragma unroll
    for (int hto = 0; hto < HT; ++hto) {
#pragma unroll
        for (int r = 0; r < 16; ++r) a[hto][r] = trelu(a[hto][r]);
        hout[hto] = a[hto];
    }
}

template <int HT, int NK>
__device__ __forceinline__ f32x16 hidden_tile(const float* __restrict__ W, int woff, int boff, int hto,
                                              const f32x16 (&hin)[HT]) {
    const int lane = lane_id(), h = lane >> 5;
    f32x16 a = load_bias16(W + boff + hto * 32, h);
#pragma unroll
    for (int kt = 0; kt < NK; ++kt) {
#pragma unroll
        for (int rq = 0; rq < 4; ++rq) {
            const f32x4 w = *reinterpret_cast<const f32x4*>(W + woff + (a_quad(a_tile(hto, kt, HT), rq) * 64 + lane) * 4);
#pragma unroll
            for (int rr = 0; rr < 4; ++rr) a = mfma32(w[rr], hin[kt][4 * rq + rr], a);
        }
    }
#pragma unroll
    for (int r = 0; r < 16; ++r) a[r] = trelu(a[r]);
    return a;
}

template <int HT, int N>
__device__ __forceinline__ f32x16 hidden_tile_n(int n, const float* __restrict__ W, int woff, int boff,
                                                int hto, const f32x16 (&hin)[HT]) {
    if constexpr (N == 0) {
        return hidden_tile<HT, 0>(W, woff, boff, hto, hin);
    } else {
        if (n >= N) return hidden_tile<HT, N>(W, woff, boff, hto, hin);
        return hidden_tile_n<HT, N - 1>(n, W, woff, boff, hto, hin);
    }
}

template <int HT>
__device__ __forceinline__ void made_hidden_nk(const float* __restrict__ W, int woff, int boff,
                                               const f32x16 (&hin)[HT], f32x16 (&hout)[HT],
                                               const int (&nk)[HT], bool full) {
    if (full) {
        made_hidden1<HT>(W, woff, boff, hin, hout);
        return;
    }
#pragma unroll
    for (int hto = 0; hto < HT; ++hto) hout[hto] = hidden_tile_n<HT, HT>(nk[hto], W, woff, boff, hto, hin);
}

template <int HT, int NK>
__device__ __forceinline__ void out_pair(const float* __restrict__ W, const MadeLayout& L, int j,
                                         const f32x16 (&hin)[HT], f32x16& mu, f32x16& al) {
    const int lane = lane_id(), h = lane >> 5;
    mu = load_bias16(W + L.b4 + (j * 2 + 0) * 32, h);
    al = load_bias16(W + L.b4 + (j * 2 + 1) * 32, h);
#pragma unroll
    for (int kt = 0; kt < NK; ++kt) {
#pragma unroll
        for (int rq = 0; rq < 4; ++rq) {
            const f32x4 wm = *reinterpret_cast<const f32x4*>(
                W + L.w4 + (a_quad(a_tile(j * 2 + 0, kt, HT), rq) * 64 + lane) * 4);
            const f32x4 wa = *reinterpret_cast<const f32x4*>(
                W + L.w4 + (a_quad(a_tile(j * 2 + 1, kt, HT), rq) * 64 + lane) * 4);
#pragma unroll
            for (int rr = 0; rr < 4; ++rr) {
                mu = mfma32(wm[rr], hin[kt][4 * rq + rr], mu);
                al = mfma32(wa[rr], hin[kt][4 * rq + rr], al);
            }
        }
    }
}

template <int HT, int N>
__device__ __forceinline__ void out_pair_n(int n, const float* __restrict__ W, const MadeLayout& L, int j,
                                           const f32x16 (&hin)[HT], f32x16& mu, f32x16& al) {
    if constexpr (N == 0) {
        out_pair<HT, 0>(W, L, j, hin, mu, al);
    } else {
        if (n >= N) {
            out_pair<HT, N>(W, L, j, hin, mu, al);
            return;
        }
        out_pair_n<HT, N - 1>(n, W, L, j, hin, mu, al);
    }
}

struct MadeDraw {
    uint64_t seed;
    uint64_t* rng;
    float* z;
};
__device__ __forceinline__ const MadeDraw& made_draw_arg(const MadeDraw& a) { return a; }
__device__ __forceinline__ void made_draw_tile(float (&pf)[32], int64_t tt, int64_t ntiles, int64_t B, int d,
                                               uint64_t seed, uint64_t off) {
    const int lane = lane_id();
    const bool live = tt < ntiles;
#pragma unroll
    for (int r = 0; r < 32; ++r) {
        const int64_t row = tt * 32 + r;
        pf[r] = 0.f;
        if (live && row < B) {
            const float v = base_value(row, lane, seed, off);
            pf[r] = lane < d ? v : 0.f;
        }
    }
}

template <int HT, bool WLDS, int VAR, bool LOGP, bool SAMPLE = false, typename... DRAW>
__global__ __launch_bounds__(512) void made_tile_kernel(
    const float* __restrict__ packed, const float* __restrict__ in, float* __restrict__ out,
    float* __restrict__ logdet, int64_t B, int d, int accumulate, int64_t ntiles,
    float* __restrict__ logp, double* __restrict__ partials, double* __restrict__ sums, float cgauss,
    DRAW... draw) {
    static_assert(sizeof...(DRAW) == (SAMPLE ? 1 : 0), "SAMPLE kernels take one MadeDraw");
    static_assert(!SAMPLE || (VAR == NFX_IAF_FORWARD && !LOGP), "SAMPLE: the IAF forward pass");
    const MadeLayout L = made_layout(d, HT);
    constexpr int S = kTileStride;
    extern __shared__ f32x4 lds4[];
    float* lds = reinterpret_cast<float*>(lds4);
    const int wave = __builtin_amdgcn_readfirstlane(threadIdx.x >> 6);
    const int nwg = LOGP ? 8 : (int)(blockDim.x >> 6);
    if constexpr (WLDS) {
        const f32x4* src = reinterpret_cast<const f32x4*>(packed);
        for (int i = threadIdx.x; i < L.par_total / 4; i += 64 * nwg) lds4[i] = src[i];
    }
    float* xt = lds + (WLDS ? L.par_total : 0) + wave * 32 * S;
    if constexpr (WLDS) __syncthreads();
    const int lane = lane_id(), h = lane >> 5, col = lane & 31;
    const int64_t nwaves = (int64_t)gridDim.x * nwg;
    const int voff = lane < d ? lane * 4 : (1 << 30);
    const int rowb = d * 4;
    const int* nkp = reinterpret_cast<const int*>(packed);
    int nk1[HT], nk2[HT], nk3[HT];
    bool full2 = true, full3 = true;
#pragma unroll
    for (int i = 0; i < HT; ++i) {
        nk1[i] = nkp[L.nk1 + i];
        nk2[i] = nkp[L.nk2 + i];
        nk3[i] = nkp[L.nk3 + i];
        full2 = full2 && nk2[i] >= HT;
        full3 = full3 && nk3[i] >= HT;
    }
    const float tsafe = packed[L.tsafe];

    int64_t t = (int64_t)blockIdx.x * nwg + wave;
    double lpacc = 0.0;
    float pf[32];
    float ldpf = 0.f;
    uint64_t draw_off = 0;
    if constexpr (SAMPLE) {
        draw_off = rng_offset(made_draw_arg(draw...).rng);
        made_draw_tile(pf, t, ntiles, B, d, made_draw_arg(draw...).seed, draw_off);
    } else {
        if (accumulate && t < ntiles && lane < 32 && t * 32 + col < B) ldpf = logdet[t * 32 + col];
        const int64_t rows = t < ntiles ? (B - t * 32 < 32 ? B - t * 32 : 32) : 0;
        const auto rs = __builtin_amdgcn_make_buffer_rsrc(const_cast<float*>(in) + (t < ntiles ? t * 32 * d : 0), 0,
                                                          (int)(rows * rowb), 0x00020000);
#pragma unroll
        for (int r = 0; r < 32; ++r)
            pf[r] = __uint_as_float(__builtin_amdgcn_raw_buffer_load_b32(rs, voff, r * rowb, 0));
    }
    for (; t < ntiles; t += nwaves) {
        const int64_t base = t * 32;
        const int rows = (int)(B - base < 32 ? B - base : 32);
        const float* W = (WLDS ? lds : packed) + opaque_zero();
        float xmax = 0.f;
#pragma unroll
        for (int r = 0; r < 32; ++r) {
            xt[r * S + lane] = pf[r];
            xmax = tmax(xmax, fabsf(pf[r]));
        }
        if constexpr (SAMPLE) {
            const auto rs = __builtin_amdgcn_make_buffer_rsrc(made_draw_arg(draw...).z + base * d, 0, rows * rowb,
                                                              0x00020000);
#pragma unroll
            for (int r = 0; r < 32; ++r)
                __builtin_amdgcn_raw_buffer_store_b32(__float_as_uint(pf[r]), rs, voff, r * rowb, 0);
        }
        const bool dense = __builtin_amdgcn_ballot_w64(!(xmax <= tsafe)) != 0;
        wave_lds_sync();

        f32x16 h1[HT];
#pragma unroll
        for (int ht = 0; ht < HT; ++ht) {
            f32x16 a = load_bias16(W + L.b1 + ht * 32, h);
            const int nkc = dense ? L.NKC : nk1[ht];
            for (int kc = 0; kc < nkc; ++kc) {
#pragma unroll
                for (int g = 0; g < 4; ++g) {
                    const f32x4 w =
                        *reinterpret_cast<const f32x4*>(W + L.w1 + ((ht * 4 * L.NKC + kc * 4 + g) * 64 + lane) * 4);
#pragma unroll
                    for (int rr = 0; rr < 4; ++rr) a = mfma32(w[rr], xt[col * S + 32 * kc + 8 * g + 2 * rr + h], a);
                }
            }
#pragma unroll
            for (int r = 0; r < 16; ++r) a[r] = trelu(a[r]);
            h1[ht] = a;
        }
        f32x16 h2[HT];
        made_hidden_nk<HT>(W, L.w2, L.b2, h1, h2, nk2, dense || full2);
        made_hidden_nk<HT>(W, L.w3, L.b3, h2, h1, nk3, dense || full3);

        const float ldin = ldpf;
        if constexpr (SAMPLE) {
            made_draw_tile(pf, t + nwaves, ntiles, B, d, made_draw_arg(draw...).seed, draw_off);
        } else {
            const int64_t tn = t + nwaves;
            ldpf = (accumulate && tn < ntiles && lane < 32 && tn * 32 + col < B) ? logdet[tn * 32 + col] : 0.f;
            const int64_t rn = tn < ntiles ? (B - tn * 32 < 32 ? B - tn * 32 : 32) : 0;
            const auto rs = __builtin_amdgcn_make_buffer_rsrc(const_cast<float*>(in) + (tn < ntiles ? tn * 32 * d : 0), 0,
                                                              (int)(rn * rowb), 0x00020000);
#pragma unroll
            for (int r = 0; r < 32; ++r)
                pf[r] = __uint_as_float(__builtin_amdgcn_raw_buffer_load_b32(rs, voff, r * rowb, 0));
        }

        float acc = 0.f;
        for (int j = 0; j < L.NJ; ++j) {
            f32x16 mu, al;
            out_pair_n<HT, HT>(dense ? HT : nkp[L.nk4 + j], W, L, j, h1, mu, al);
#pragma unroll
            for (int r = 0; r < 16; ++r) {
                float* p = xt + col * S + 32 * j + crow(r, h);
                *p = made_affine<VAR>(*p, mu[r], al[r], acc);
            }
        }
        const float ssum = halves_sum(acc, acc);
        wave_lds_sync();
        float zsq = 0.f;
        if constexpr (LOGP) {
            if (lane < 32) {
                for (int jd = 0; jd < d; ++jd) {
                    const float v = xt[col * S + jd];
                    zsq = (jd == 0) ? gauss_sq0(v) : gauss_sq(zsq, v);
                }
            }
        }
        {
            const auto rs = __builtin_amdgcn_make_buffer_rsrc(out + base * d, 0, rows * rowb, 0x00020000);
#pragma unroll
            for (int r = 0; r < 32; ++r)
                __builtin_amdgcn_raw_buffer_store_b32(__float_as_uint(xt[r * S + lane]), rs, voff, r * rowb, 0);
        }
        if (lane < 32 && col < rows) {
            float ldv;
            if constexpr (VAR == NFX_MAF_INVERSE) {
                ldv = -ssum;
                if (nonfinite(ldv)) ldv = 0.f;
                ldv = tclamp(ldv, -100.f, 100.f);
            } else {
                ldv = ssum;
                if (nonfinite(ldv)) ldv = 0.f;
                ldv = tclamp(ldv, -50.f, 50.f);
            }
            const int64_t so = base + col;
            const float ldt = accumulate ? ldin + ldv : ldv;
            logdet[so] = ldt;
            if constexpr (LOGP) {
                const float lp = gauss_lp(zsq, cgauss, ldt);
                logp[so] = lp;
                lpacc += (double)lp;
            }
        }
        wave_lds_sync();
    }
    if constexpr (LOGP) {
        logp_commit<512>(lpacc, partials, sums, B);
    }
    if constexpr (SAMPLE) {
        rng_commit(made_draw_arg(draw...).rng);
    }
}

typedef void (*made_par_kernel_t)(const float*, const float*, float*, float*, int64_t, int, int, int64_t,
                                  float*, double*, double*, float);

template <int HT>
made_par_kernel_t made_pick_ht(bool wlds, int variant);
template <int HT>
made_par_kernel_t made_tile_pick_ht(bool wlds, int variant, bool logp);
template <int HT>
made_seq_kernel_t made_seq_pick_ht(int variant);
typedef void (*made_sample_kernel_t)(const float*, const float*, float*, float*, int64_t, int, int, int64_t, float*,
                                     double*, double*, float, MadeDraw);
template <int HT>
made_sample_kernel_t made_tile_sample_pick_ht(bool wlds);

}
```

### normalizing-flows-study_amd/csrc/nfx_made_sample.hip

```cpp
#include "nfx_made_kernel.h"

namespace nfx {

template <int HT>
made_sample_kernel_t made_tile_sample_pick_ht(bool wlds) {
    return wlds ? made_tile_kernel<HT, true, NFX_IAF_FORWARD, false, true, MadeDraw>
                : made_tile_kernel<HT, false, NFX_IAF_FORWARD, false, true, MadeDraw>;
}
template made_sample_kernel_t made_tile_sample_pick_ht<1>(bool);
template made_sample_kernel_t made_tile_sample_pick_ht<2>(bool);
template made_sample_kernel_t made_tile_sample_pick_ht<3>(bool);
template made_sample_kernel_t made_tile_sample_pick_ht<4>(bool);

}
```

### normalizing-flows-study_amd/csrc/nfx_pack.h

```cpp
#pragma once
#include "nfx_common.h"

namespace nfx {

__device__ inline float mlp_weight(const NfxMlpRaw& net, int layer, int in_dim, int row, int col) {
    size_t idx = (size_t)row * in_dim + col;
    float w = net.w[layer][idx];
    if (net.mask[layer]) w = w * net.mask[layer][idx];
    if (layer < 3 && net.bn_w[layer]) {
        double a = (double)net.bn_w[layer][row] / sqrt((double)net.bn_rv[layer][row] + (double)net.bn_eps);
        return (float)(a * (double)w);
    }
    return w;
}

__device__ inline float mlp_bias(const NfxMlpRaw& net, int layer, int row) {
    float b = net.b[layer] ? net.b[layer][row] : 0.f;
    if (layer < 3 && net.bn_w[layer]) {
        double a = (double)net.bn_w[layer][row] / sqrt((double)net.bn_rv[layer][row] + (double)net.bn_eps);
        return (float)(a * ((double)b - (double)net.bn_rm[layer][row]) + (double)net.bn_b[layer][row]);
    }
    return b;
}

__device__ inline double block_mlp_tsafe(const NfxMlpRaw& net, int nl, const int* rows, const int* cols,
                                         double lim, double* red ) {
    double alpha = 1.0, beta = 0.0, tsafe = 3.0e38;
    for (int l = 0; l < nl; ++l) {
        double nmax = 0.0, cmax = 0.0;
        for (int r0 = 0; r0 < rows[l]; r0 += (int)(blockDim.x >> 3)) {
            const int r = r0 + (threadIdx.x >> 3), q = threadIdx.x & 7;
            double sum = 0.0;
            if (r < rows[l])
                for (int c = q; c < cols[l]; c += 8) sum += fabs((double)mlp_weight(net, l, cols[l], r, c));
            sum += __shfl_xor(sum, 1);
            sum += __shfl_xor(sum, 2);
            sum += __shfl_xor(sum, 4);
            if (r < rows[l]) {
                nmax = (sum > nmax || sum != sum) ? sum : nmax;
                const double b = fabs((double)mlp_bias(net, l, r));
                cmax = (b > cmax || b != b) ? b : cmax;
            }
        }
        auto nmaxd = [](double a, double b) { return (b > a || b != b) ? b : a; };
#pragma unroll
        for (int o = 32; o > 0; o >>= 1) {
            nmax = nmaxd(nmax, __shfl_xor(nmax, o));
            cmax = nmaxd(cmax, __shfl_xor(cmax, o));
        }
        const int wv = threadIdx.x >> 6;
        if ((threadIdx.x & 63) == 0) {
            red[2 * wv] = nmax;
            red[2 * wv + 1] = cmax;
        }
        __syncthreads();
        nmax = red[0];
        cmax = red[1];
        for (int w = 1; w < (int)(blockDim.x >> 6); ++w) {
            nmax = nmaxd(nmax, red[2 * w]);
            cmax = nmaxd(cmax, red[2 * w + 1]);
        }
        __syncthreads();
        alpha = nmax * alpha;
        beta = nmax * beta + cmax;
        if (!(beta < lim) || !(alpha < 1e300)) tsafe = 0.0;
        else if (alpha > 0.0) tsafe = fmin(tsafe, (lim - beta) / alpha);
    }
    return tsafe;
}

}
```

### normalizing-flows-study_amd/nfs_amd/_lib.py

```python
import ctypes
import os
import threading
import types

import torch

_HERE = os.path.dirname(os.path.abspath(__file__))
LIB_PATH = os.environ.get("NFX_LIB", os.path.join(_HERE, "libnfx.so"))

NFX_OK = 0
NFX_EINVAL = -1
NFX_EUNSUPPORTED = -2
NFX_ELAUNCH = -3
NFX_FORWARD = 1
NFX_INVERSE = -1
NFX_MAF_INVERSE = 0
NFX_IAF_FORWARD = 1
NFX_MAF_FORWARD = 2
NFX_IAF_INVERSE = 3
NFX_AFFINE_AUTO = 0
NFX_AFFINE_STREAMING = 1
NFX_AFFINE_SMALL = 2
NFX_MADE_SEQ_AUTO = 0
NFX_MADE_SEQ_SEGMENT = 1
NFX_MADE_SEQ_WAVE = 2
NFX_MADE_SEQ_PUSH = 3
NFX_RESIDUAL_RELU = 0
NFX_RESIDUAL_ELU = 1
NFX_RESIDUAL_LEAKY_RELU = 2
NFX_RESIDUAL_TANH = 3
NFX_NAF_RELU = 0
NFX_NAF_ELU = 1
NFX_NAF_LEAKY_RELU = 2
NFX_NAF_GELU = 3
NFX_NAF_LAYER_NORM = 1


def NFX_NAF_RESIDUAL(l):
    return 2 << l


class NfxLibraryError(RuntimeError):
    pass


class NfxError(RuntimeError):
    pass


class NfxMlpRaw(ctypes.Structure):
    _fields_ = [
        ("w", ctypes.c_void_p * 4),
        ("b", ctypes.c_void_p * 4),
        ("mask", ctypes.c_void_p * 4),
        ("bn_w", ctypes.c_void_p * 3),
        ("bn_b", ctypes.c_void_p * 3),
        ("bn_rm", ctypes.c_void_p * 3),
        ("bn_rv", ctypes.c_void_p * 3),
        ("bn_eps", ctypes.c_float),
        ("n_layers", ctypes.c_int),
    ]


class NfxNafLayer(ctypes.Structure):
    _fields_ = [
        ("weight", ctypes.c_void_p),
        ("bias", ctypes.c_void_p),
        ("mask", ctypes.c_void_p),
        ("ln_weight", ctypes.c_void_p),
        ("ln_bias", ctypes.c_void_p),
        ("ln_eps", ctypes.c_float),
        ("residual", ctypes.c_int),
    ]


class NfxNafLayerGrad(ctypes.Structure):
    _fields_ = [
        ("weight", ctypes.c_void_p),
        ("bias", ctypes.c_void_p),
        ("ln_weight", ctypes.c_void_p),
        ("ln_bias", ctypes.c_void_p),
    ]


_vp = ctypes.c_void_p
_i64 = ctypes.c_int64
_int = ctypes.c_int
_f = ctypes.c_float
_sz = ctypes.c_size_t

_SIGNATURES = {
    "nfx_abi_version": (_int, []),
    "nfx_last_error": (ctypes.c_char_p, []),
    "nfx_last_kernel": (ctypes.c_char_p, []),
    "nfx_debug_fill_lds": (ctypes.c_int, [ctypes.c_uint32, ctypes.c_void_p]),
    "nfx_affine_packed_floats": (_sz, [_int, _int]),
    "nfx_affine_pack": (_int, [ctypes.POINTER(NfxMlpRaw), ctypes.POINTER(NfxMlpRaw), _vp, _int, _int, _vp, _vp]),
    "nfx_affine_coupling": (_int, [_vp, _vp, _vp, _vp, _i64, _int, _int, _int, _int, _vp]),
    "nfx_affine_coupling_logprob": (_int, [_vp, _vp, _vp, _vp, _vp, _vp, _vp, _i64, _int, _int, _int, _vp]),
    "nfx_affine_kernel_policy": (_int, [_int]),
    "nfx_linear_forward": (_int, [_vp, _vp, _vp, _vp, _vp, _vp, _vp, _vp, _i64, _int, _int, _int, _vp]),
    "nfx_linear_backward_data": (_int, [_vp, _vp, _vp, _vp, _vp, _vp, _i64, _int, _int, _int, _vp]),
    "nfx_linear_workspace_bytes": (_sz, [_i64, _int, _int]),
    "nfx_linear_backward_weight": (_int, [_vp, _vp, _vp, _vp, _vp, _vp, _i64, _int, _int, _vp, _vp]),
    "nfx_made_elem_forward": (_int, [_vp, _vp, _vp, _vp, _i64, _int, _int, _int, _vp]),
    "nfx_made_elem_step": (_int, [_vp, _vp, _vp, _vp, _i64, _int, _int, _int, _vp]),
    "nfx_made_elem_finish": (_int, [_vp, _vp, _vp, _vp, _vp, _i64, _int, _int, _int, _vp]),
    "nfx_made_elem_backward": (_int, [_vp, _vp, _vp, _vp, _vp, _vp, _i64, _int, _int, _vp]),
    "nfx_made_elem_seq_backward": (_int, [_vp, _vp, _vp, _vp, _vp, _vp, _vp, _i64, _int, _int, _int, _vp]),
    "nfx_made_elem_seq_step_backward": (_int, [_vp, _vp, _vp, _vp, _vp, _vp, _vp, _vp, _vp, _i64, _int, _int, _int,
                                               _vp]),
    "nfx_made_elem_prefix": (_int, [_vp, _vp, _i64, _int, _int, _vp]),
    "nfx_affine_elem_forward": (_int, [_vp, _vp, _vp, _vp, _vp, _vp, _i64, _int, _int, _int, _vp]),
    "nfx_affine_elem_backward": (_int, [_vp, _vp, _vp, _vp, _vp, _vp, _vp, _vp, _vp, _i64, _int, _int, _vp]),
    "nfx_bn_prepare": (_int, [_vp, _vp, _vp, _vp, _vp, ctypes.c_double, ctypes.c_double, _int, _int, _vp, _vp, _vp,
                              _vp, _vp]),
    "nfx_bn_apply_relu": (_int, [_vp, _vp, _vp, _vp, _i64, _int, _vp]),
    "nfx_arqs_step": (_int, [_vp, _vp, _vp, _vp, _vp, _vp, _vp, _vp, _i64, _int, _int, _int, _int, _int, _f, _f, _f,
                             _vp]),
    "nfx_bn_workspace_bytes": (_sz, [_i64, _int]),
    "nfx_bn_backward_sums": (_int, [_vp, _vp, _vp, _vp, _vp, _i64, _int, _vp, _vp]),
    "nfx_bn_backward_apply": (_int, [_vp, _vp, _vp, _vp, _vp, _vp, _vp, _int, _vp, _i64, _int, _vp]),
    "nfx_spline_elem_forward": (_int, [_vp, _vp, _vp, _vp, _vp, _i64, _int, _int, _f, _f, _f, _f, _int, _int, _vp]),
    "nfx_spline_elem_backward": (_int, [_vp, _vp, _vp, _vp, _vp, _vp, _vp, _i64, _int, _int, _f, _f, _f, _f, _int,
                                        _vp]),
    "nfx_spline_elem_forward_bounded": (_int, [_vp, _vp, _vp, _vp, _vp, _vp, _i64, _int, _int, _f, _f, _f, _f, _int,
                                               _int, _vp]),
    "nfx_spline_elem_backward_bounded": (_int, [_vp, _vp, _vp, _vp, _vp, _vp, _vp, _vp, _i64, _int, _int, _f, _f, _f,
                                                _f, _int, _vp]),
    "nfx_spline_rescale": (_int, [_vp, _vp, _vp, _i64, _int, _f, _vp]),
    "nfx_arqs_bounds": (_int, [_vp, _vp, _vp, _i64, _int, _int, _vp]),
    "nfx_affine_chain_supported": (_int, [_i64, _int, _int]),
    "nfx_affine_chain": (_int, [ctypes.POINTER(_vp), _int, _vp, _vp, _vp, _i64, _int, _int, _int, _int, _vp]),
    "nfx_affine_chain_logprob": (_int, [ctypes.POINTER(_vp), _int, _vp, _vp, _vp, _vp, _vp, _vp, _i64, _int, _int,
                                        _int, _vp]),
    "nfx_affine_chain_sample": (_int, [ctypes.POINTER(_vp), _int, ctypes.c_uint64, _vp, _vp, _vp, _vp, _i64, _int, _int,
                                       _vp]),
    "nfx_arqs_packed_floats": (_sz, [_int, _int, _int]),
    "nfx_arqs_pack": (_int, [ctypes.POINTER(NfxMlpRaw), _int, _int, _int, _vp, _vp]),
    "nfx_arqs": (_int, [_vp, _vp, _vp, _vp, _i64, _int, _int, _int, _f, _f, _f, _int, ctypes.c_double,
                        ctypes.c_double, _int, _int, _vp]),
    "nfx_spline_packed_floats": (_sz, [_int, _int, _int]),
    "nfx_spline_pack": (_int, [ctypes.POINTER(NfxMlpRaw), _vp, _int, _int, _int, _vp, _vp]),
    "nfx_spline_coupling": (_int, [_vp, _vp, _vp, _vp, _i64, _int, _int, _int, _f, _f, _f, _f,
                                   _int, _f, _f, _int, _int, _vp]),
    "nfx_spline_coupling_logprob": (_int, [_vp, _vp, _vp, _vp, _vp, _vp, _vp, _i64, _int, _int, _int, _f, _f,
                                           _f, _f, _int, _f, _f, _int, _vp]),
    "nfx_spline_chain_supported": (_int, [_i64, _int, _int, _int]),
    "nfx_spline_chain": (_int, [ctypes.POINTER(_vp), _int, _vp, _vp, _vp, _i64, _int, _int, _int, _f, _f, _f, _f,
                                _int, _int, _vp]),
    "nfx_spline_chain_logprob": (_int, [ctypes.POINTER(_vp), _int, _vp, _vp, _vp, _vp, _vp, _vp, _i64, _int, _int,
                                        _int, _f, _f, _f, _f, _int, _vp]),
    "nfx_spline_chain_sample": (_int, [ctypes.POINTER(_vp), _int, ctypes.c_uint64, _vp, _vp, _vp, _vp, _i64, _int, _int,
                                       _int, _f, _f, _f, _f, _vp]),
    "nfx_cnf_packed_floats": (_sz, [_int, _int]),
    "nfx_cnf_pack": (_int, [_vp, _vp, _vp, _vp, _vp, _vp, _int, _int, _vp, _vp]),
    "nfx_cnf_supported": (_int, [_i64, _int, _int]),
    "nfx_cnf_integrate": (_int, [_vp, _vp, _vp, _vp, _i64, _int, _int, _f, _f, _f, _int, _vp]),
    "nfx_cnf_backward_supported": (_int, [_i64, _int, _int]),
    "nfx_cnf_backward_packed_floats": (_sz, [_int, _int]),
    "nfx_cnf_trajectory_floats": (_sz, [_i64, _int, _f, _f, _f]),
    "nfx_cnf_backward_workspace_floats": (_sz, [_i64, _int, _int]),
    "nfx_cnf_backward_slots": (_sz, [_i64, _int, _int]),
    "nfx_cnf_backward_block_threads": (_sz, [_i64, _int, _int]),
    "nfx_cnf_pack_backward": (_int, [_vp, _vp, _vp, _vp, _vp, _vp, _int, _int, _vp, _vp]),
    "nfx_cnf_integrate_save": (_int, [_vp, _vp, _vp, _vp, _vp, _i64, _int, _int, _f, _f, _f, _int, _vp]),
    "nfx_cnf_backward": (_int, [_vp] * 16 + [_i64, _int, _int, _f, _f, _f, _vp]),
    "nfx_residual_packed_floats": (_sz, [_int, _int]),
    "nfx_residual_supported": (_int, [_i64, _int, _int, _int]),
    "nfx_residual_pack": (_int, [_vp, _vp, _vp, _vp, _f] * 3 + [_int, _int, _vp, _vp]),
    "nfx_residual_flow": (_int, [_vp, _vp, _vp, _vp, _i64, _int, _int, _int, _int, _int, _int, _f, _int, _vp]),
    "nfx_residual_backward_supported": (_int, [_i64, _int, _int, _int]),
    "nfx_residual_backward_packed_floats": (_sz, [_int, _int]),
    "nfx_residual_backward_workspace_floats": (_sz, [_i64, _int, _int]),
    "nfx_residual_backward_slots": (_sz, [_i64, _int, _int]),
    "nfx_residual_backward_block_threads": (_sz, [_i64, _int, _int]),
    "nfx_residual_pack_backward": (_int, [_vp, _vp, _vp, _vp, _f] * 3 + [_int, _int, _vp, _vp]),
    "nfx_residual_backward": (_int, [_vp] * 12 + [_i64, _int, _int, _int, _int, _int, _vp]),
    "nfx_naf_packed_floats": (_sz, [_int, _int, _vp]),
    "nfx_naf_supported": (_int, [_i64, _int, _int, _vp, _int, _int]),
    "nfx_naf_pack": (_int, [_vp, _int, _int, _vp, _vp, _vp]),
    "nfx_naf_flow": (_int, [_vp, _vp, _vp, _vp, _i64, _int, _int, _vp, _int, _int, _f, _f, _int, _int, _vp]),
    "nfx_naf_backward_supported": (_int, [_i64, _int, _int, _vp, _int, _int]),
    "nfx_naf_backward_packed_floats": (_sz, [_int, _int, _vp]),
    "nfx_naf_pack_backward": (_int, [_vp, _int, _int, _vp, _vp, _vp]),
    "nfx_naf_backward_slots": (_sz, [_i64, _int, _int, _vp]),
    "nfx_naf_backward_block_threads": (_sz, [_i64, _int, _int, _vp]),
    "nfx_naf_backward_workspace_floats": (_sz, [_i64, _int, _int, _vp]),
    "nfx_naf_backward": (_int, [_vp] * 8 + [_i64, _int, _int, _vp, _int, _int, _f, _f, _vp]),
    "nfx_lowrank_supported": (_int, [_i64, _int, _int]),
    "nfx_lowrank_record_floats": (_sz, [_int]),
    "nfx_lowrank_pack_planar": (_int, [_vp, _vp, _vp, _int, _int, _f, _vp, _vp]),
    "nfx_lowrank_pack_radial": (_int, [_vp, _vp, _vp, _int, _int, _f, _vp, _vp]),
    "nfx_lowrank_pack_sylvester": (_int, [_vp, _vp, _vp, _int, _int, _int, _int, _f, _vp, _vp]),
    "nfx_lowrank_stack": (_int, [_vp, _int, _vp, _vp, _vp, _i64, _int, _int, _int, _vp]),
    "nfx_lrbwd_supported": (_int, [_i64, _int, _int, _int]),
    "nfx_lrbwd_max_layers": (_sz, [_int]),
    "nfx_lrbwd_chunk_rows": (_sz, [_int]),
    "nfx_lrbwd_slots": (_sz, [_i64, _int, _int]),
    "nfx_lrbwd_workspace_floats": (_sz, [_i64, _int, _int]),
    "nfx_lrbwd_stack": (_int, [_vp, _int, _vp, _vp, _vp, _vp, _vp, _i64, _int, _int, _vp]),
    "nfx_lrbwd_param_grads": (_int, [_vp, _i64, _int, _int, _int, _int, _vp, _vp, _vp, _vp, _vp, _vp, _int, _int, _vp]),
    "nfx_rqs_unit": (_int, [_vp, _vp, _vp, _vp, _vp, _vp, _i64, _int, _f, _f, _f, _int, _vp]),
    "nfx_rqs_unit_backward": (_int, [_vp, _vp, _vp, _vp, _vp, _vp, _vp, _vp, _vp, _vp, _i64, _int, _f, _f, _f, _int,
                                     _vp]),
    "nfx_made_packed_floats": (_sz, [_int, _int]),
    "nfx_made_pack": (_int, [ctypes.POINTER(NfxMlpRaw), _int, _int, _vp, _vp]),
    "nfx_made_pack_parallel": (_int, [ctypes.POINTER(NfxMlpRaw), _int, _int, _vp, _vp]),
    "nfx_made_pack_sequential": (_int, [_int, _int, _vp, _vp]),
    "nfx_made_seq_policy": (_int, [_int]),
    "nfx_base_normal": (_int, [ctypes.c_uint64, _vp, _vp, _i64, _int, _vp]),
    "nfx_made_sample_supported": (_int, [_int, _int, _int]),
    "nfx_made_affine_sample": (_int, [_vp, ctypes.c_uint64, _vp, _vp, _vp, _vp, _i64, _int, _int, _vp]),
    "nfx_made_affine": (_int, [_vp, _vp, _vp, _vp, _i64, _int, _int, _int, _int, _vp]),
    "nfx_made_affine_logprob": (_int, [_vp, _vp, _vp, _vp, _vp, _vp, _vp, _i64, _int, _int, _int, _int, _vp]),
    "nfx_made_pack_backward": (_int, [ctypes.POINTER(NfxMlpRaw), _int, _int, _vp, _vp]),
    "nfx_made_backward_factor_floats": (_sz, [_i64, _int, _int]),
    "nfx_made_backward_max_batch": (_i64, [_int, _int]),
    "nfx_made_affine_backward": (_int, [_vp, _vp, _vp, _vp, _vp, _vp, _i64, _int, _int, _int, _vp]),
    "nfx_made_seq_backward": (_int, [_vp, _vp, _vp, _vp, _vp, _vp, _i64, _int, _int, _int, _vp]),
    "nfx_made_factor_pitch": (_i64, [_i64]),
    "nfx_made_param_floats": (_sz, [_int, _int]),
    "nfx_made_wgrad_workspace_bytes": (_sz, [_i64, _int, _int]),
    "nfx_made_backward_weights": (_int, [_vp, _i64, _int, _int, ctypes.POINTER(_vp), _vp, _vp, _vp]),
    "nfx_affine_train_pack_floats": (_sz, [_int, _int]),
    "nfx_affine_train_stats_doubles": (_sz, [_int]),
    "nfx_affine_train_grad_doubles": (_sz, [_int, _int]),
    "nfx_affine_train_param_floats": (_sz, [_int, _int]),
    "nfx_affine_train_workspace_bytes": (_sz, [_i64, _int, _int]),
    "nfx_affine_train_pack": (_int, [ctypes.POINTER(NfxMlpRaw), ctypes.POINTER(NfxMlpRaw), _vp, _vp, _vp, _int,
                                     _int, _vp, _vp, _vp]),
    "nfx_affine_train_stats": (_int, [_vp, _vp, _i64, _int, _int, _int, _vp, _vp, _vp]),
    "nfx_affine_train_update_running": (_int, [_vp, _vp, ctypes.POINTER(_vp), ctypes.POINTER(_vp), _int,
                                               ctypes.c_double, _vp]),
    "nfx_affine_train_update_running_counted": (_int, [_vp, _vp, ctypes.POINTER(_vp), ctypes.POINTER(_vp),
                                                       ctypes.POINTER(_vp), _int, ctypes.c_double, _vp]),
    "nfx_affine_train_backward": (_int, [_vp, _vp, _vp, _vp, _vp, _i64, _int, _int, _int, _int, _vp, _vp, _vp,
                                         _vp]),
    "nfx_affine_train_assemble": (_int, [_vp, _vp, _vp, _int, _int, _f, _vp, _vp]),
    "nfx_affine_train_keep_floats": (_sz, [_i64, _int, _int]),
    "nfx_affine_train_stats_keep": (_int, [_vp, _vp, _i64, _int, _int, _int, _vp, _vp, _vp, _vp]),
    "nfx_affine_train_backward_keep": (_int, [_vp, _vp, _vp, _vp, _vp, _i64, _int, _int, _int, _int, _vp, _vp,
                                              _vp, _vp, _vp]),
    "nfx_affine_train_output": (_int, [_vp, _vp, _vp, _vp, _vp, _i64, _int, _int, _int, _vp]),
    "nfx_affine_eval_stats": (_int, [ctypes.POINTER(_vp), ctypes.POINTER(_vp), _int, _vp, _vp, _vp]),
    "nfx_spline_backward_packed_floats": (_sz, [_int, _int, _int]),
    "nfx_spline_backward_param_floats": (_sz, [_int, _int, _int]),
    "nfx_spline_backward_workspace_bytes": (_sz, [_i64, _int, _int, _int]),
    "nfx_spline_pack_backward": (_int, [ctypes.POINTER(NfxMlpRaw), _vp, _int, _int, _int, _vp, _vp]),
    "nfx_spline_coupling_backward": (_int, [_vp, _vp, _vp, _vp, _vp, _vp, _vp, _vp, _i64, _int, _int, _int, _int,
                                            _f, _f, _f, _f, _int, _vp]),
    "nfx_gauss_workspace_bytes": (_sz, [_i64]),
    "nfx_gauss_workspace_init": (_int, [_vp, _vp]),
    "nfx_gauss_logprob": (_int, [_vp, _vp, _vp, _vp, _vp, _i64, _int, _vp]),
    "nfx_gauss_logprob_backward": (_int, [_vp, _vp, _vp, _vp, _i64, _int, _vp]),
    "nfx_flowbn_workspace_bytes": (_sz, [_i64, _int]),
    "nfx_flowbn_apply": (_int, [_vp, _vp, _vp, _vp, _vp, _vp, _vp, _f, _i64, _int, _int, _vp]),
    "nfx_flowbn_moments": (_int, [_vp, _i64, _int, _vp, _vp, _vp]),
    "nfx_flowbn_update_running": (_int, [_vp, _vp, _vp, ctypes.c_double, _int, _vp]),
    "nfx_flowbn_backward": (_int, [_vp, _vp, _vp, _vp, _vp, _vp, _vp, _vp, _f, _vp, _vp, _i64, _int, _int,
                                   _vp, _vp]),
}

EXPORTED_SYMBOLS = tuple(_SIGNATURES)

_VALUE_RETURNING = frozenset((
    "nfx_abi_version", "nfx_affine_kernel_policy", "nfx_made_seq_policy", "nfx_affine_chain_supported",
    "nfx_spline_chain_supported", "nfx_cnf_supported", "nfx_cnf_backward_supported",
    "nfx_made_sample_supported", "nfx_residual_supported", "nfx_residual_backward_supported",
    "nfx_naf_supported", "nfx_naf_backward_supported",
    "nfx_lowrank_supported", "nfx_lrbwd_supported"))


_as_pointer = _vp.from_param


class DevicePtr:

    @staticmethod
    def from_param(v):
        if v is None or type(v) is int:
            return _as_pointer(v)
        return _as_pointer(v.data_ptr())


def _raise_on_status(rc, fn, args):
    if rc != NFX_OK:
        raise NfxError(f"{fn.__name__} failed (rc={rc}): {lib().nfx_last_error().decode(errors='replace')}")
    return rc


_lock = threading.Lock()
_lib = None
_checked = None


def load(path=LIB_PATH):
    global _lib, _checked
    with _lock:
        if _lib is not None:
            return _lib
        if not os.path.exists(path):
            raise NfxLibraryError(
                f"libnfx.so not found at {path}: build it with "
                f"`python normalizing-flows-study_amd/build.py` (or __graft_entry__.build()). "
                f"The HIP path has no eager fallback.")
        l = ctypes.CDLL(path)
        n = types.SimpleNamespace()
        for name, (res, args) in _SIGNATURES.items():
            fn = getattr(l, name, None)
            if fn is None:
                continue
            fn.restype = res
            fn.argtypes = args
            cf = l._FuncPtr((name, l))
            cf.__name__ = name
            cf.restype = res
            cf.argtypes = [DevicePtr if a is _vp else a for a in args]
            if res is _int and name not in _VALUE_RETURNING:
                cf.errcheck = _raise_on_status
            setattr(n, name, cf)
        _checked = n
        _lib = l
        return l


def lib():
    l = _lib
    return l if l is not None else load()


def checked():
    if _checked is None:
        load()
    return _checked


def available():
    try:
        load()
        return True
    except NfxLibraryError:
        return False


def check(rc, what):
    if rc != NFX_OK:
        msg = lib().nfx_last_error().decode(errors="replace")
        raise NfxError(f"{what} failed (rc={rc}): {msg}")


def dense(t):
    t = t.contiguous()
    if t.data_ptr() & 15:
        t = t.clone()
    return t


def ptr(t):
    return None if t is None else t.data_ptr()


try:
    _raw_stream = torch._C._cuda_getCurrentRawStream
except AttributeError:
    _raw_stream = None


def stream_of(t):
    if _raw_stream is not None and t.device.type == "cuda":
        return _raw_stream(t.device.index if t.device.index is not None else torch.cuda.current_device())
    return torch.cuda.current_stream(t.device).cuda_stream


def mlp_raw(linears, batchnorms=(), masks=None):
    raw = NfxMlpRaw()
    keep = []

    def p(t):
        t = dense(t.detach().float())
        keep.append(t)
        return t.data_ptr()

    raw.n_layers = len(linears)
    for i, lin in enumerate(linears):
        raw.w[i] = p(lin.weight)
        raw.b[i] = p(lin.bias) if lin.bias is not None else None
        if masks is not None and masks[i] is not None:
            raw.mask[i] = p(masks[i])
    eps = 1e-5
    for i, bn in enumerate(batchnorms):
        if bn is None:
            continue
        raw.bn_w[i] = p(bn.weight) if bn.weight is not None else p(torch.ones_like(bn.running_var))
        raw.bn_b[i] = p(bn.bias) if bn.bias is not None else p(torch.zeros_like(bn.running_var))
        raw.bn_rm[i] = p(bn.running_mean)
        raw.bn_rv[i] = p(bn.running_var)
        eps = bn.eps
    raw.bn_eps = eps
    return raw, keep


def last_kernel():
    return lib().nfx_last_kernel().decode()
```

Measured before the change: 1.615 billion.

## Add bf16x3 split-precision MFMA path for MADE tile kernel

Adds a split-precision path for the MADE tile kernel at small shapes (HT<=2, d<=64). Weights are pre-split into three bf16 parts and packed into compact live blocks, and activations are split on the fly so the hidden layers run on bf16 MFMA with six cross terms instead of the fp32 MFMA path. The pack step computes per-layer norm bounds and a validity flag so rows outside a safe range can fall back. It adds pack-time work, more kernel instantiations and a risk of accuracy drift against the fp32 NLL.

```diff
diff --git a/include/nfx.h b/include/nfx.h
--- a/include/nfx.h
+++ b/include/nfx.h
@@ -119,6 +119,9 @@
 #define NFX_MADE_SEQ_WAVE 2
 #define NFX_MADE_SEQ_PUSH 3
 int nfx_made_seq_policy(int policy);
+#define NFX_MADE_TILE_AUTO 0
+#define NFX_MADE_TILE_FP32 1
+int nfx_made_tile_policy(int policy);
 int nfx_made_affine_logprob(const float* packed, const float* in, float* out, float* log_det,
                             float* logp, double* sums, void* workspace, int64_t B, int d, int H,
                             int variant, int accumulate, void* stream);
diff --git a/normalizing-flows-study_amd/csrc/nfx_affine_kernel.h b/normalizing-flows-study_amd/csrc/nfx_affine_kernel.h
--- a/normalizing-flows-study_amd/csrc/nfx_affine_kernel.h
+++ b/normalizing-flows-study_amd/csrc/nfx_affine_kernel.h
@@ -3,6 +3,7 @@
 #include <utility>
 
 #include "nfx_common.h"
+#include "nfx_split.h"
 
 namespace nfx {
 
@@ -150,39 +151,6 @@
         res[j] = tclamp(halves_sum(part[j][0], part[j][1]) + P[L.b3 + j], -10.f, 10.f);
 }
 
-#ifndef NFX_SPLIT_TERMS
-#define NFX_SPLIT_TERMS 6
-#endif
-typedef __bf16 bf16x8 __attribute__((ext_vector_type(8)));
-typedef uint32_t u32x4 __attribute__((ext_vector_type(4)));
-
-__device__ __forceinline__ f32x16 mfma_bf16(u32x4 a, u32x4 b, f32x16 c) {
-    return __builtin_amdgcn_mfma_f32_32x32x16_bf16(__builtin_bit_cast(bf16x8, a), __builtin_bit_cast(bf16x8, b), c,
-                                                    0, 0, 0);
-}
-
-__device__ __forceinline__ void split3(float x, uint32_t& u0, uint32_t& u1, uint32_t& u2) {
-    u0 = __float_as_uint(x) & 0xffff0000u;
-    const float r1 = x - __uint_as_float(u0);
-    u1 = __float_as_uint(r1) & 0xffff0000u;
-    u2 = __float_as_uint(r1 - __uint_as_float(u1));
-}
-
-__device__ __forceinline__ uint32_t pack_bf16(uint32_t lo, uint32_t hi) {
-    return __builtin_amdgcn_perm(hi, lo, 0x07060302u);
-}
-
-__device__ __forceinline__ void split_block(const f32x16& a, int half, u32x4 (&xp)[3]) {
-#pragma unroll
-    for (int q = 0; q < 4; ++q) {
-        uint32_t l0, l1, l2, h0, h1, h2;
-        split3(a[8 * half + 2 * q], l0, l1, l2);
-        split3(a[8 * half + 2 * q + 1], h0, h1, h2);
-        xp[0][q] = pack_bf16(l0, h0);
-        xp[1][q] = pack_bf16(l1, h1);
-        xp[2][q] = pack_bf16(l2, h2);
-    }
-}
 
 template <class F, int... I>
 __device__ __forceinline__ void static_for_seq(F&& f, std::integer_sequence<int, I...>) {
@@ -192,12 +160,6 @@
 __device__ __forceinline__ void static_for(F&& f) {
     static_for_seq(f, std::make_integer_sequence<int, N>{});
 }
-
-#if NFX_SPLIT_TERMS == 8
-constexpr int kSplitTermW[8] = {2, 1, 2, 1, 0, 1, 0, 0}, kSplitTermX[8] = {1, 2, 0, 1, 2, 0, 1, 0};
-#else
-constexpr int kSplitTermW[6] = {2, 1, 0, 1, 0, 0}, kSplitTermX[6] = {0, 1, 2, 0, 1, 0};
-#endif
 
 template <int HT, int D, int TILES, bool LIVE>
 __device__ __forceinline__ void affine_nets_split_pipe(const float* __restrict__ S, const AffineSplit& SL,
diff --git a/normalizing-flows-study_amd/csrc/nfx_made.hip b/normalizing-flows-study_amd/csrc/nfx_made.hip
--- a/normalizing-flows-study_amd/csrc/nfx_made.hip
+++ b/normalizing-flows-study_amd/csrc/nfx_made.hip
@@ -101,8 +101,90 @@
     for (int i = threadIdx.x; i < 3 * HT + L.NJ; i += kLiveThreads) nk[L.nk1 + i] = 0;
     __shared__ double red[256];
     const int rows[4] = {H, H, H, 2 * d}, cols[4] = {d, H, H, H};
-    const double tsafe = block_mlp_tsafe(net, 4, rows, cols, 1.0e37, red);
+    double norms[8];
+    const double tsafe = block_mlp_tsafe(net, 4, rows, cols, 1.0e37, red, norms);
     if (threadIdx.x == 0) packed[L.tsafe] = (float)fmin(tsafe, 3.0e38);
+    if (made_has_split(d, HT) && threadIdx.x == 0) {
+        double alpha = 1.0, beta = 0.0, xs = 3.0e38, tail = 1.0, worst = 0.0;
+        for (int l = 0; l < 4; ++l) {
+            alpha = norms[2 * l] * alpha;
+            beta = norms[2 * l] * beta + norms[2 * l + 1];
+            if (!(beta < 1.0e30) || !(alpha < 1e300)) xs = 0.0;
+            else if (alpha > 0.0) xs = fmin(xs, (1.0e30 - beta) / alpha);
+        }
+        bool lost = false;
+        for (int l = 3; l >= 0; --l) {
+            tail = tail * norms[2 * l];
+            worst = fmax(worst, tail);
+            lost = lost || !(tail < 1e300);
+        }
+        lost = lost || !(0x1p-133 * worst < 0x1p-24);
+        packed[L.sp_ok] = (!lost && xs > 0.0) ? 1.f : 0.f;
+        packed[L.sp_ok + 1] = (float)xs;
+    }
+}
+
+__global__ __launch_bounds__(1024) void made_split_pack_kernel(int d, int H, float* packed) {
+    const int HT = (H + 31) / 32;
+    const MadeLayout L = made_layout(d, HT);
+    const int Hp = L.Hp, maxb = made_split_max_blocks(d, HT);
+    const int* nk = reinterpret_cast<const int*>(packed);
+    __shared__ int w_bad;
+    if (threadIdx.x == 0) w_bad = 0;
+    __syncthreads();
+    for (int i = threadIdx.x; i < L.sp_w - L.sp_b; i += blockDim.x) {
+        const int nb = 3 * HT * 32;
+        const int src = i < HT * 32 ? L.b1 + i : i < 2 * HT * 32 ? L.b2 + (i - HT * 32)
+                        : i < nb ? L.b3 + (i - 2 * HT * 32) : L.b4 + (i - nb);
+        packed[L.sp_b + i] = packed[src];
+    }
+    int nlive = 0;
+    for (int i = 0; i < 3 * HT; ++i) nlive += nk[L.nk1 + i];
+    for (int j = 0; j < L.NJ; ++j) nlive += 2 * nk[L.nk4 + j];
+    bool bad = false;
+    for (int i = threadIdx.x; i < maxb * kSplitBlockDwords; i += blockDim.x) {
+        int rem = i / kSplitBlockDwords, layer = -1, ot = 0, kt = 0;
+        for (int l = 0; l < 3 && layer < 0; ++l)
+            for (int ht = 0; ht < HT && layer < 0; ++ht) {
+                const int n = nk[L.nk1 + l * HT + ht];
+                if (rem < n) { layer = l; ot = ht; kt = rem; } else rem -= n;
+            }
+        for (int j = 0; j < L.NJ && layer < 0; ++j) {
+            const int n = nk[L.nk4 + j];
+            if (rem < 2 * n) { layer = 3; ot = 2 * j + (rem >= n ? 1 : 0); kt = rem % n; } else rem -= 2 * n;
+        }
+        const int t = i % kSplitBlockDwords, q = t & 3, lane = (t >> 2) & 63, p = (t >> 8) % 3, kb = t / 768;
+        const int row = lane & 31, h = lane >> 5;
+        uint32_t half[2] = {0u, 0u};
+        for (int e = 0; e < 2 && layer >= 0; ++e) {
+            const int el = 2 * q + e;
+            float w;
+            if (layer == 0) {
+                const int k = 32 * kt + 16 * kb + 8 * h + el, a = 32 * ot + row;
+                w = k < d ? packed[L.s_w1t + k * Hp + a] : 0.f;
+            } else {
+                const int k = 32 * kt + crow(8 * kb + el, h);
+                if (layer < 3) {
+                    w = packed[(layer == 1 ? L.s_w2 : L.s_w3) + (32 * ot + row) * Hp + k];
+                } else {
+                    const int orow = 32 * (ot >> 1) + row;
+                    w = orow < d ? packed[L.s_w4 + ((ot & 1) * d + orow) * Hp + k] : 0.f;
+                }
+            }
+            if (!(fabsf(w) <= 1e6f)) bad = true;
+            uint32_t u[3];
+            split_weight3(w, u);
+            half[e] = u[p];
+        }
+        packed[L.sp_w + i] = __uint_as_float(half[0] | (half[1] << 16));
+    }
+    if (bad) atomicOr(&w_bad, 1);
+    __syncthreads();
+    if (threadIdx.x == 0) {
+        if (w_bad || nlive > maxb) packed[L.sp_ok] = 0.f;
+        reinterpret_cast<int*>(packed)[L.sp_ok + 2] = nlive;
+        packed[L.sp_ok + 3] = 0.f;
+    }
 }
 
 __global__ __launch_bounds__(256) void made_extent_kernel(int d, int H, float* packed) {
@@ -161,7 +243,8 @@
     return pick_range<1, 4>(HT, [=](auto HT_) { return made_pick_ht<HT_()>(wlds, variant); });
 }
 
-static made_par_kernel_t pick_tile(int HT, bool wlds, int variant, bool logp) {
+static made_par_kernel_t pick_tile(int HT, bool wlds, int variant, bool logp, bool split) {
+    if (split) return pick_range<1, 2>(HT, [=](auto HT_) { return made_tile_split_pick_ht<HT_()>(wlds, variant, logp); });
     return pick_range<1, 4>(HT, [=](auto HT_) { return made_tile_pick_ht<HT_()>(wlds, variant, logp); });
 }
 
@@ -222,8 +305,11 @@
         const MadeLayout L = made_layout(d, HT);
         const int groups = HT * 4 * L.NKC + 2 * HT * HT * 4 + L.NJ * 2 * HT * 4;
         made_extent_kernel<<<(groups + 3) / 4, 256, 0, (hipStream_t)stream>>>(d, H, packed);
-    }
-    return check_launch("made_extent_kernel");
+        rc = check_launch("made_extent_kernel");
+        if (rc || !made_has_split(d, HT)) return rc;
+    }
+    made_split_pack_kernel<<<1, 1024, 0, (hipStream_t)stream>>>(d, H, packed);
+    return check_launch("made_split_pack_kernel");
 }
 
 extern "C" int nfx_made_pack_sequential(int d, int H, float* packed, void* stream) {
@@ -269,10 +355,23 @@
     bool wlds;
     size_t lds;
 };
-static TileConfig tile_config(const MadeLayout& L, int64_t ntiles, bool fused) {
+static std::atomic<int>& made_tile_policy() {
+    static std::atomic<int> v{[] {
+        const char* e = getenv("NFX_MADE_TILE_POLICY");
+        return e ? atoi(e) : NFX_MADE_TILE_AUTO;
+    }()};
+    return v;
+}
+static bool tile_split(int d, int HT) {
+    return made_has_split(d, HT) && made_tile_policy().load(std::memory_order_relaxed) != NFX_MADE_TILE_FP32;
+}
+
+static TileConfig tile_config(const MadeLayout& L, int64_t ntiles, bool fused, bool split) {
     int nw = 8;
     if (!fused && ntiles < 4 * (int64_t)num_cus()) nw = (int)((ntiles + num_cus() - 1) / num_cus());
-    const size_t wbytes = (size_t)L.par_total * sizeof(float);
+    const size_t wfloats =
+        split ? (size_t)(L.sp_w - L.sp_b) + (size_t)made_split_max_blocks(L.d, L.HT) * kSplitBlockDwords : (size_t)L.par_total;
+    const size_t wbytes = wfloats * sizeof(float);
     const size_t tiles = nw * 32 * (size_t)kTileStride * sizeof(float);
     const bool wlds = nw == 8 && wbytes + tiles <= kLdsBytes;
     return {nw, wlds, (wlds ? wbytes : 0) + tiles};
@@ -323,8 +422,9 @@
     }
     if (tile_path(d, HT, variant)) {
         const int64_t ntiles = (B + 31) / 32;
-        const TileConfig c = tile_config(L, ntiles, fused);
-        made_par_kernel_t k = pick_tile(HT, c.wlds, variant, fused);
+        const bool split = tile_split(d, HT);
+        const TileConfig c = tile_config(L, ntiles, fused, split);
+        made_par_kernel_t k = pick_tile(HT, c.wlds, variant, fused, split);
         if (!k) return set_error(NFX_EUNSUPPORTED, "made_affine: no kernel for H=%d", H);
         int rc = prepare_lds((const void*)k, c.lds);
         if (rc) return rc;
@@ -388,6 +488,12 @@
     return made_seq_policy().exchange(policy);
 }
 
+extern "C" int nfx_made_tile_policy(int policy) {
+    if (policy < 0) return made_tile_policy().load();
+    if (policy > NFX_MADE_TILE_FP32) return set_error(NFX_EINVAL, "made_tile_policy: unknown policy %d", policy);
+    return made_tile_policy().exchange(policy);
+}
+
 extern "C" int nfx_made_affine(const float* packed, const float* in, float* out, float* log_det,
                                int64_t B, int d, int H, int variant, int accumulate, void* stream) {
     return made_launch(packed, in, out, log_det, B, d, H, variant, accumulate, nullptr, nullptr, nullptr,
@@ -418,9 +524,11 @@
     const int HT = (H + 31) / 32;
     const MadeLayout L = made_layout(d, HT);
     const int64_t ntiles = (B + 31) / 32;
-    const TileConfig c = tile_config(L, ntiles, false);
+    const bool split = tile_split(d, HT);
+    const TileConfig c = tile_config(L, ntiles, false, split);
     made_sample_kernel_t k =
-        pick_range<1, 4>(HT, [=](auto HT_) { return made_tile_sample_pick_ht<HT_()>(c.wlds); });
+        split ? pick_range<1, 2>(HT, [=](auto HT_) { return made_tile_split_sample_pick_ht<HT_()>(c.wlds); })
+              : pick_range<1, 4>(HT, [=](auto HT_) { return made_tile_sample_pick_ht<HT_()>(c.wlds); });
     int rc = prepare_lds((const void*)k, c.lds);
     if (rc) return rc;
     int grid = resident_grid((const void*)k, 64 * c.nw, c.lds, (ntiles + c.nw - 1) / c.nw);
diff --git a/normalizing-flows-study_amd/csrc/nfx_made_kernel.h b/normalizing-flows-study_amd/csrc/nfx_made_kernel.h
--- a/normalizing-flows-study_amd/csrc/nfx_made_kernel.h
+++ b/normalizing-flows-study_amd/csrc/nfx_made_kernel.h
@@ -1,6 +1,7 @@
 #pragma once
 #include "nfx_common.h"
 #include "nfx_rng.h"
+#include "nfx_split.h"
 
 namespace nfx {
 
@@ -15,8 +16,18 @@
     int sw1, sw4, sb4;
     int ctab;
     int ps, pw4, pw1, pb4, pw23, ptb, ptab;
+    int sp_b, sp_w, sp_ok;
     int total;
 };
+
+constexpr int kSplitBlockDwords = 2 * 3 * 256;
+constexpr int kSplitMaxD = 64;
+__host__ __device__ constexpr bool made_has_split(int d, int HT) { return HT <= 2 && d <= kSplitMaxD; }
+__host__ __device__ constexpr int made_split_max_blocks(int d, int HT) {
+    const int NK = (d + 31) / 32;
+    const int dense = HT * NK + 2 * HT * HT + NK * 2 * HT;
+    return dense < 15 ? dense : 15;
+}
 
 __host__ __device__ constexpr int made_up4(int v) { return (v + 3) & ~3; }
 
@@ -80,6 +91,11 @@
     L.pw23 = o; o += PS ? 2 * L.Hp * L.Hp : 0;
     L.ptb = o; o += PS ? 4 * L.Hp : 0;
     L.ptab = o; o += PS ? 16 * seqp_max_chunks(d, L.Hp) : 0;
+    const bool SP = made_has_split(d, HT);
+    o = made_up4(o);
+    L.sp_b = o; o += SP ? 3 * HT * 32 + L.NJ * 64 : 0;
+    L.sp_w = o; o += SP ? made_split_max_blocks(d, HT) * kSplitBlockDwords : 0;
+    L.sp_ok = o; o += SP ? 4 : 0;
     L.total = o;
     return L;
 }
@@ -528,7 +544,70 @@
     }
 }
 
-template <int HT, bool WLDS, int VAR, bool LOGP, bool SAMPLE = false, typename... DRAW>
+template <int HT>
+__device__ __forceinline__ void tile_hidden_fp32(const float* __restrict__ W, const MadeLayout& L, const float* xt,
+                                                 const int (&nk1)[HT], const int (&nk2)[HT], const int (&nk3)[HT],
+                                                 bool dense, bool full2, bool full3, f32x16 (&h1)[HT]) {
+    constexpr int S = kTileStride;
+    const int lane = lane_id(), h = lane >> 5, col = lane & 31;
+#pragma unroll
+    for (int ht = 0; ht < HT; ++ht) {
+        f32x16 a = load_bias16(W + L.b1 + ht * 32, h);
+        const int nkc = dense ? L.NKC : nk1[ht];
+        for (int kc = 0; kc < nkc; ++kc) {
+#pragma unroll
+            for (int g = 0; g < 4; ++g) {
+                const f32x4 w =
+                    *reinterpret_cast<const f32x4*>(W + L.w1 + ((ht * 4 * L.NKC + kc * 4 + g) * 64 + lane) * 4);
+#pragma unroll
+                for (int rr = 0; rr < 4; ++rr) a = mfma32(w[rr], xt[col * S + 32 * kc + 8 * g + 2 * rr + h], a);
+            }
+        }
+#pragma unroll
+        for (int r = 0; r < 16; ++r) a[r] = trelu(a[r]);
+        h1[ht] = a;
+    }
+    f32x16 h2[HT];
+    made_hidden_nk<HT>(W, L.w2, L.b2, h1, h2, nk2, dense || full2);
+    made_hidden_nk<HT>(W, L.w3, L.b3, h2, h1, nk3, dense || full3);
+}
+
+
+__device__ __forceinline__ void split_x_block(const float* xrow, u32x4 (&xp)[3]) {
+#pragma unroll
+    for (int q = 0; q < 4; ++q) {
+        uint32_t l0, l1, l2, h0, h1, h2;
+        split3(xrow[2 * q], l0, l1, l2);
+        split3(xrow[2 * q + 1], h0, h1, h2);
+        xp[0][q] = pack_bf16(l0, h0);
+        xp[1][q] = pack_bf16(l1, h1);
+        xp[2][q] = pack_bf16(l2, h2);
+    }
+}
+
+template <int NKT>
+__device__ __forceinline__ f32x16 split_tile(const u32x4* __restrict__ wp, int blk, int nkt,
+                                             const float* __restrict__ bias, const u32x4 (&xp)[2 * NKT][3]) {
+    f32x16 hi = load_bias16(bias, lane_id() >> 5), lo = {};
+#pragma unroll
+    for (int kt = 0; kt < NKT; ++kt) {
+        if (kt < nkt) {
+#pragma unroll
+            for (int kb = 0; kb < 2; ++kb) {
+                const u32x4* w = wp + ((blk + kt) * 6 + kb * 3) * 64;
+                const u32x4 wv[3] = {w[0], w[64], w[128]};
+#pragma unroll
+                for (int t = 0; t < NFX_SPLIT_TERMS; ++t) {
+                    if (t + 1 < NFX_SPLIT_TERMS) lo = mfma_bf16(wv[kSplitTermW[t]], xp[2 * kt + kb][kSplitTermX[t]], lo);
+                    else hi = mfma_bf16(wv[kSplitTermW[t]], xp[2 * kt + kb][kSplitTermX[t]], hi);
+                }
+            }
+        }
+    }
+    return hi + lo;
+}
+
+template <int HT, bool WLDS, int VAR, bool LOGP, bool SAMPLE = false, bool SPLIT = false, typename... DRAW>
 __global__ __launch_bounds__(512) void made_tile_kernel(
     const float* __restrict__ packed, const float* __restrict__ in, float* __restrict__ out,
     float* __restrict__ logdet, int64_t B, int d, int accumulate, int64_t ntiles,
@@ -536,18 +615,20 @@
     DRAW... draw) {
     static_assert(sizeof...(DRAW) == (SAMPLE ? 1 : 0), "SAMPLE kernels take one MadeDraw");
     static_assert(!SAMPLE || (VAR == NFX_IAF_FORWARD && !LOGP), "SAMPLE: the IAF forward pass");
+    static_assert(!SPLIT || HT <= 2, "SPLIT: made_has_split shapes");
     const MadeLayout L = made_layout(d, HT);
     constexpr int S = kTileStride;
     extern __shared__ f32x4 lds4[];
     float* lds = reinterpret_cast<float*>(lds4);
     const int wave = __builtin_amdgcn_readfirstlane(threadIdx.x >> 6);
     const int nwg = LOGP ? 8 : (int)(blockDim.x >> 6);
-    if constexpr (WLDS) {
+    if constexpr (WLDS && !SPLIT) {
         const f32x4* src = reinterpret_cast<const f32x4*>(packed);
         for (int i = threadIdx.x; i < L.par_total / 4; i += 64 * nwg) lds4[i] = src[i];
     }
-    float* xt = lds + (WLDS ? L.par_total : 0) + wave * 32 * S;
-    if constexpr (WLDS) __syncthreads();
+    const int sp_floats = (L.sp_w - L.sp_b) + made_split_max_blocks(d, HT) * kSplitBlockDwords;
+    float* xt = lds + (WLDS ? (SPLIT ? sp_floats : L.par_total) : 0) + wave * 32 * S;
+    if constexpr (WLDS && !SPLIT) __syncthreads();
     const int lane = lane_id(), h = lane >> 5, col = lane & 31;
     const int64_t nwaves = (int64_t)gridDim.x * nwg;
     const int voff = lane < d ? lane * 4 : (1 << 30);
@@ -564,6 +645,28 @@
         full3 = full3 && nk3[i] >= HT;
     }
     const float tsafe = packed[L.tsafe];
+    [[maybe_unused]] int bo1[HT], bo2[HT], bo3[HT], bo4 = 0;
+    [[maybe_unused]] bool use_split = false;
+    [[maybe_unused]] float xsafe = 0.f;
+    if constexpr (SPLIT) {
+        int nb = 0;
+#pragma unroll
+        for (int i = 0; i < HT; ++i) { bo1[i] = nb; nb += nk1[i]; }
+#pragma unroll
+        for (int i = 0; i < HT; ++i) { bo2[i] = nb; nb += nk2[i]; }
+#pragma unroll
+        for (int i = 0; i < HT; ++i) { bo3[i] = nb; nb += nk3[i]; }
+        bo4 = nb;
+        for (int j = 0; j < L.NJ; ++j) nb += 2 * nkp[L.nk4 + j];
+        use_split = packed[L.sp_ok] != 0.f && nb <= made_split_max_blocks(d, HT);
+        xsafe = packed[L.sp_ok + 1];
+        if constexpr (WLDS) {
+            const int n4 = use_split ? ((L.sp_w - L.sp_b) + nb * kSplitBlockDwords) / 4 : 0;
+            const f32x4* src = reinterpret_cast<const f32x4*>(packed + L.sp_b);
+            for (int i = threadIdx.x; i < n4; i += 64 * nwg) lds4[i] = src[i];
+            __syncthreads();
+        }
+    }
 
     int64_t t = (int64_t)blockIdx.x * nwg + wave;
     double lpacc = 0.0;
@@ -585,7 +688,7 @@
     for (; t < ntiles; t += nwaves) {
         const int64_t base = t * 32;
         const int rows = (int)(B - base < 32 ? B - base : 32);
-        const float* W = (WLDS ? lds : packed) + opaque_zero();
+        const float* W = ((WLDS && !SPLIT) ? lds : packed) + opaque_zero();
         float xmax = 0.f;
 #pragma unroll
         for (int r = 0; r < 32; ++r) {
@@ -602,50 +705,107 @@
         const bool dense = __builtin_amdgcn_ballot_w64(!(xmax <= tsafe)) != 0;
         wave_lds_sync();
 
-        f32x16 h1[HT];
-#pragma unroll
-        for (int ht = 0; ht < HT; ++ht) {
-            f32x16 a = load_bias16(W + L.b1 + ht * 32, h);
-            const int nkc = dense ? L.NKC : nk1[ht];
-            for (int kc = 0; kc < nkc; ++kc) {
-#pragma unroll
-                for (int g = 0; g < 4; ++g) {
-                    const f32x4 w =
-                        *reinterpret_cast<const f32x4*>(W + L.w1 + ((ht * 4 * L.NKC + kc * 4 + g) * 64 + lane) * 4);
-#pragma unroll
-                    for (int rr = 0; rr < 4; ++rr) a = mfma32(w[rr], xt[col * S + 32 * kc + 8 * g + 2 * rr + h], a);
-                }
-            }
-#pragma unroll
-            for (int r = 0; r < 16; ++r) a[r] = trelu(a[r]);
-            h1[ht] = a;
-        }
-        f32x16 h2[HT];
-        made_hidden_nk<HT>(W, L.w2, L.b2, h1, h2, nk2, dense || full2);
-        made_hidden_nk<HT>(W, L.w3, L.b3, h2, h1, nk3, dense || full3);
-
-        const float ldin = ldpf;
-        if constexpr (SAMPLE) {
-            made_draw_tile(pf, t + nwaves, ntiles, B, d, made_draw_arg(draw...).seed, draw_off);
+        float ldin = 0.f;
+        auto prefetch = [&]() {
+            ldin = ldpf;
+            if constexpr (SAMPLE) {
+                made_draw_tile(pf, t + nwaves, ntiles, B, d, made_draw_arg(draw...).seed, draw_off);
+            } else {
+                const int64_t tn = t + nwaves;
+                ldpf = (accumulate && tn < ntiles && lane < 32 && tn * 32 + col < B) ? logdet[tn * 32 + col] : 0.f;
+                const int64_t rn = tn < ntiles ? (B - tn * 32 < 32 ? B - tn * 32 : 32) : 0;
+                const auto rs = __builtin_amdgcn_make_buffer_rsrc(
+                    const_cast<float*>(in) + (tn < ntiles ? tn * 32 * d : 0), 0, (int)(rn * rowb), 0x00020000);
+#pragma unroll
+                for (int r = 0; r < 32; ++r)
+                    pf[r] = __uint_as_float(__builtin_amdgcn_raw_buffer_load_b32(rs, voff, r * rowb, 0));
+            }
+        };
+        float acc = 0.f;
+        auto out_fp32 = [&](const f32x16 (&h3)[HT], bool dns, bool take) {
+            for (int j = 0; j < L.NJ; ++j) {
+                f32x16 mu, al;
+                out_pair_n<HT, HT>(dns ? HT : nkp[L.nk4 + j], W, L, j, h3, mu, al);
+#pragma unroll
+                for (int r = 0; r < 16; ++r) {
+                    float* p = xt + col * S + 32 * j + crow(r, h);
+                    if (take) *p = made_affine<VAR>(*p, mu[r], al[r], acc);
+                }
+            }
+        };
+
+        if constexpr (!SPLIT) {
+            f32x16 h1[HT];
+            tile_hidden_fp32<HT>(W, L, xt, nk1, nk2, nk3, dense, full2, full3, h1);
+            prefetch();
+            out_fp32(h1, dense, true);
         } else {
-            const int64_t tn = t + nwaves;
-            ldpf = (accumulate && tn < ntiles && lane < 32 && tn * 32 + col < B) ? logdet[tn * 32 + col] : 0.f;
-            const int64_t rn = tn < ntiles ? (B - tn * 32 < 32 ? B - tn * 32 : 32) : 0;
-            const auto rs = __builtin_amdgcn_make_buffer_rsrc(const_cast<float*>(in) + (tn < ntiles ? tn * 32 * d : 0), 0,
-                                                              (int)(rn * rowb), 0x00020000);
-#pragma unroll
-            for (int r = 0; r < 32; ++r)
-                pf[r] = __uint_as_float(__builtin_amdgcn_raw_buffer_load_b32(rs, voff, r * rowb, 0));
-        }
-
-        float acc = 0.f;
-        for (int j = 0; j < L.NJ; ++j) {
-            f32x16 mu, al;
-            out_pair_n<HT, HT>(dense ? HT : nkp[L.nk4 + j], W, L, j, h1, mu, al);
-#pragma unroll
-            for (int r = 0; r < 16; ++r) {
-                float* p = xt + col * S + 32 * j + crow(r, h);
-                *p = made_affine<VAR>(*p, mu[r], al[r], acc);
+            bool mybad = !use_split;
+            if (!use_split || __builtin_amdgcn_ballot_w64(!(xmax <= xsafe)) != 0) {
+                if (use_split) {
+                    bool bad = false;
+                    for (int k = 0; k < 32; ++k) bad = bad || !(fabsf(xt[col * S + 32 * h + k]) <= xsafe);
+                    const uint64_t m = __builtin_amdgcn_ballot_w64(bad);
+                    mybad = (((uint32_t)m | (uint32_t)(m >> 32)) >> col) & 1u;
+                    wave_lds_sync();
+                }
+                const bool dns = use_split || dense;
+                f32x16 h1[HT];
+                tile_hidden_fp32<HT>(W, L, xt, nk1, nk2, nk3, dns, full2, full3, h1);
+                out_fp32(h1, dns, mybad);
+                wave_lds_sync();
+            }
+            if (use_split) {
+                const float* SB = (WLDS ? lds : packed + L.sp_b) + opaque_zero();
+                const u32x4* SW = reinterpret_cast<const u32x4*>(SB + (L.sp_w - L.sp_b)) + lane;
+                f32x16 hh[HT];
+                {
+                    u32x4 xp[4][3];
+#pragma unroll
+                    for (int kb = 0; kb < 4; ++kb) {
+                        if (kb < 2 * L.NKC) {
+                            split_x_block(xt + col * S + 16 * kb + 8 * h, xp[kb]);
+                        } else {
+#pragma unroll
+                            for (int p = 0; p < 3; ++p) xp[kb][p] = u32x4{0u, 0u, 0u, 0u};
+                        }
+                    }
+#pragma unroll
+                    for (int ht = 0; ht < HT; ++ht) hh[ht] = split_tile<2>(SW, bo1[ht], nk1[ht], SB + ht * 32, xp);
+                }
+                u32x4 xp[2 * HT][3];
+                auto split_act = [&]() {
+#pragma unroll
+                    for (int ht = 0; ht < HT; ++ht) {
+#pragma unroll
+                        for (int r = 0; r < 16; ++r) hh[ht][r] = trelu(hh[ht][r]);
+                        split_block(hh[ht], 0, xp[2 * ht]);
+                        split_block(hh[ht], 1, xp[2 * ht + 1]);
+                    }
+                };
+                split_act();
+#pragma unroll
+                for (int ht = 0; ht < HT; ++ht) hh[ht] = split_tile<HT>(SW, bo2[ht], nk2[ht], SB + (HT + ht) * 32, xp);
+                split_act();
+#pragma unroll
+                for (int ht = 0; ht < HT; ++ht)
+                    hh[ht] = split_tile<HT>(SW, bo3[ht], nk3[ht], SB + (2 * HT + ht) * 32, xp);
+                split_act();
+                prefetch();
+                int blk = bo4;
+                for (int j = 0; j < L.NJ; ++j) {
+                    const int n4 = nkp[L.nk4 + j];
+                    const f32x16 mu = split_tile<HT>(SW, blk, n4, SB + 3 * HT * 32 + (2 * j) * 32, xp);
+                    const f32x16 al = split_tile<HT>(SW, blk + n4, n4, SB + 3 * HT * 32 + (2 * j + 1) * 32, xp);
+                    blk += 2 * n4;
+#pragma unroll
+                    for (int r = 0; r < 16; ++r) {
+                        float* p = xt + col * S + 32 * j + crow(r, h);
+                        if (!mybad) *p = made_affine<VAR>(*p, mu[r], al[r], acc);
+                    }
+                }
+            } else {
+                prefetch();
             }
         }
         const float ssum = halves_sum(acc, acc);
@@ -708,5 +868,9 @@
                                      double*, double*, float, MadeDraw);
 template <int HT>
 made_sample_kernel_t made_tile_sample_pick_ht(bool wlds);
-
-}
+template <int HT>
+made_par_kernel_t made_tile_split_pick_ht(bool wlds, int variant, bool logp);
+template <int HT>
+made_sample_kernel_t made_tile_split_sample_pick_ht(bool wlds);
+
+}
diff --git a/normalizing-flows-study_amd/csrc/nfx_made_sample.hip b/normalizing-flows-study_amd/csrc/nfx_made_sample.hip
--- a/normalizing-flows-study_amd/csrc/nfx_made_sample.hip
+++ b/normalizing-flows-study_amd/csrc/nfx_made_sample.hip
@@ -4,8 +4,8 @@
 
 template <int HT>
 made_sample_kernel_t made_tile_sample_pick_ht(bool wlds) {
-    return wlds ? made_tile_kernel<HT, true, NFX_IAF_FORWARD, false, true, MadeDraw>
-                : made_tile_kernel<HT, false, NFX_IAF_FORWARD, false, true, MadeDraw>;
+    return wlds ? made_tile_kernel<HT, true, NFX_IAF_FORWARD, false, true, false, MadeDraw>
+                : made_tile_kernel<HT, false, NFX_IAF_FORWARD, false, true, false, MadeDraw>;
 }
 template made_sample_kernel_t made_tile_sample_pick_ht<1>(bool);
 template made_sample_kernel_t made_tile_sample_pick_ht<2>(bool);
diff --git a/normalizing-flows-study_amd/csrc/nfx_made_split.hip b/normalizing-flows-study_amd/csrc/nfx_made_split.hip
--- /dev/null
+++ b/normalizing-flows-study_amd/csrc/nfx_made_split.hip
@@ -0,0 +1,27 @@
+#include "nfx_made_kernel.h"
+
+namespace nfx {
+
+template <int HT, bool WLDS>
+static made_par_kernel_t tile_split_var(int variant, bool logp) {
+    if (variant != NFX_MAF_INVERSE) return made_tile_kernel<HT, WLDS, NFX_IAF_FORWARD, false, false, true>;
+    return logp ? made_tile_kernel<HT, WLDS, NFX_MAF_INVERSE, true, false, true>
+                : made_tile_kernel<HT, WLDS, NFX_MAF_INVERSE, false, false, true>;
+}
+
+template <int HT>
+made_par_kernel_t made_tile_split_pick_ht(bool wlds, int variant, bool logp) {
+    return wlds ? tile_split_var<HT, true>(variant, logp) : tile_split_var<HT, false>(variant, logp);
+}
+template made_par_kernel_t made_tile_split_pick_ht<1>(bool, int, bool);
+template made_par_kernel_t made_tile_split_pick_ht<2>(bool, int, bool);
+
+template <int HT>
+made_sample_kernel_t made_tile_split_sample_pick_ht(bool wlds) {
+    return wlds ? made_tile_kernel<HT, true, NFX_IAF_FORWARD, false, true, true, MadeDraw>
+                : made_tile_kernel<HT, false, NFX_IAF_FORWARD, false, true, true, MadeDraw>;
+}
+template made_sample_kernel_t made_tile_split_sample_pick_ht<1>(bool);
+template made_sample_kernel_t made_tile_split_sample_pick_ht<2>(bool);
+
+}
diff --git a/normalizing-flows-study_amd/csrc/nfx_pack.h b/normalizing-flows-study_amd/csrc/nfx_pack.h
--- a/normalizing-flows-study_amd/csrc/nfx_pack.h
+++ b/normalizing-flows-study_amd/csrc/nfx_pack.h
@@ -24,7 +24,8 @@
 }
 
 __device__ inline double block_mlp_tsafe(const NfxMlpRaw& net, int nl, const int* rows, const int* cols,
-                                         double lim, double* red ) {
+                                         double lim, double* red ,
+                                         double* norms = nullptr) {
     double alpha = 1.0, beta = 0.0, tsafe = 3.0e38;
     for (int l = 0; l < nl; ++l) {
         double nmax = 0.0, cmax = 0.0;
@@ -61,6 +62,10 @@
             cmax = nmaxd(cmax, red[2 * w + 1]);
         }
         __syncthreads();
+        if (norms) {
+            norms[2 * l] = nmax;
+            norms[2 * l + 1] = cmax;
+        }
         alpha = nmax * alpha;
         beta = nmax * beta + cmax;
         if (!(beta < lim) || !(alpha < 1e300)) tsafe = 0.0;
diff --git a/normalizing-flows-study_amd/csrc/nfx_split.h b/normalizing-flows-study_amd/csrc/nfx_split.h
--- /dev/null
+++ b/normalizing-flows-study_amd/csrc/nfx_split.h
@@ -0,0 +1,53 @@
+#pragma once
+#include "nfx_common.h"
+
+namespace nfx {
+
+#ifndef NFX_SPLIT_TERMS
+#define NFX_SPLIT_TERMS 6
+#endif
+typedef __bf16 bf16x8 __attribute__((ext_vector_type(8)));
+typedef uint32_t u32x4 __attribute__((ext_vector_type(4)));
+
+__device__ __forceinline__ f32x16 mfma_bf16(u32x4 a, u32x4 b, f32x16 c) {
+    return __builtin_amdgcn_mfma_f32_32x32x16_bf16(__builtin_bit_cast(bf16x8, a), __builtin_bit_cast(bf16x8, b), c,
+                                                    0, 0, 0);
+}
+
+__device__ __forceinline__ void split3(float x, uint32_t& u0, uint32_t& u1, uint32_t& u2) {
+    u0 = __float_as_uint(x) & 0xffff0000u;
+    const float r1 = x - __uint_as_float(u0);
+    u1 = __float_as_uint(r1) & 0xffff0000u;
+    u2 = __float_as_uint(r1 - __uint_as_float(u1));
+}
+
+__device__ __forceinline__ uint32_t pack_bf16(uint32_t lo, uint32_t hi) {
+    return __builtin_amdgcn_perm(hi, lo, 0x07060302u);
+}
+
+__device__ __forceinline__ void split_block(const f32x16& a, int half, u32x4 (&xp)[3]) {
+#pragma unroll
+    for (int q = 0; q < 4; ++q) {
+        uint32_t l0, l1, l2, h0, h1, h2;
+        split3(a[8 * half + 2 * q], l0, l1, l2);
+        split3(a[8 * half + 2 * q + 1], h0, h1, h2);
+        xp[0][q] = pack_bf16(l0, h0);
+        xp[1][q] = pack_bf16(l1, h1);
+        xp[2][q] = pack_bf16(l2, h2);
+    }
+}
+
+#if NFX_SPLIT_TERMS == 8
+constexpr int kSplitTermW[8] = {2, 1, 2, 1, 0, 1, 0, 0}, kSplitTermX[8] = {1, 2, 0, 1, 2, 0, 1, 0};
+#else
+constexpr int kSplitTermW[6] = {2, 1, 0, 1, 0, 0}, kSplitTermX[6] = {0, 1, 2, 0, 1, 0};
+#endif
+
+__device__ __forceinline__ void split_weight3(float w, uint32_t (&u)[3]) {
+    u[0] = __builtin_bit_cast(uint16_t, (__bf16)w);
+    const float r1 = w - __uint_as_float(u[0] << 16);
+    u[1] = __builtin_bit_cast(uint16_t, (__bf16)r1);
+    u[2] = __builtin_bit_cast(uint16_t, (__bf16)(r1 - __uint_as_float(u[1] << 16)));
+}
+
+}
diff --git a/normalizing-flows-study_amd/nfs_amd/_lib.py b/normalizing-flows-study_amd/nfs_amd/_lib.py
--- a/normalizing-flows-study_amd/nfs_amd/_lib.py
+++ b/normalizing-flows-study_amd/nfs_amd/_lib.py
@@ -25,6 +25,8 @@
 NFX_MADE_SEQ_SEGMENT = 1
 NFX_MADE_SEQ_WAVE = 2
 NFX_MADE_SEQ_PUSH = 3
+NFX_MADE_TILE_AUTO = 0
+NFX_MADE_TILE_FP32 = 1
 NFX_RESIDUAL_RELU = 0
 NFX_RESIDUAL_ELU = 1
 NFX_RESIDUAL_LEAKY_RELU = 2
@@ -209,6 +211,7 @@
     "nfx_made_pack_parallel": (_int, [ctypes.POINTER(NfxMlpRaw), _int, _int, _vp, _vp]),
     "nfx_made_pack_sequential": (_int, [_int, _int, _vp, _vp]),
     "nfx_made_seq_policy": (_int, [_int]),
+    "nfx_made_tile_policy": (_int, [_int]),
     "nfx_base_normal": (_int, [ctypes.c_uint64, _vp, _vp, _i64, _int, _vp]),
     "nfx_made_sample_supported": (_int, [_int, _int, _int]),
     "nfx_made_affine_sample": (_int, [_vp, ctypes.c_uint64, _vp, _vp, _vp, _vp, _i64, _int, _int, _vp]),
@@ -265,7 +268,8 @@
 EXPORTED_SYMBOLS = tuple(_SIGNATURES)
 
 _VALUE_RETURNING = frozenset((
-    "nfx_abi_version", "nfx_affine_kernel_policy", "nfx_made_seq_policy", "nfx_affine_chain_supported",
+    "nfx_abi_version", "nfx_affine_kernel_policy", "nfx_made_seq_policy", "nfx_made_tile_policy",
+    "nfx_affine_chain_supported",
     "nfx_spline_chain_supported", "nfx_cnf_supported", "nfx_cnf_backward_supported",
     "nfx_made_sample_supported", "nfx_residual_supported", "nfx_residual_backward_supported",
     "nfx_naf_supported", "nfx_naf_backward_supported",
```

After: 1.612 billion. Within noise of the previous version (-0.2%).
